# Cheng-Lin-Li/show-attend-and-tell

Hardware: AMD Instinct MI355X
Metric: training images/sec (higher is better)
Workload: dtype bf16; 1 GPU; model=vgg16_frozen+attention_lstm512, global_batch=32, seq_len=20, vocab=5000, parallelism=dp1

## Files before the change

### sat_amd/ops/csrc/bptt_fuse.hip

```cpp

#include "common.h"


__global__ void lstm_in_fuse_kernel(const bf16* __restrict__ pooled,
                                    const bf16* __restrict__ table,
                                    const int64_t* __restrict__ ids,
                                    const bf16* __restrict__ sth,
                                    const int64_t* __restrict__ seed_p,
                                    bf16* __restrict__ xh,
                                    int B, int D, int E, int H,
                                    float p, int salt) {
    const uint32_t seed = (uint32_t)(*seed_p);
    const int I = D + E;
    const int W = I + H;
    int64_t idx = (int64_t)blockIdx.x * blockDim.x + threadIdx.x;
    if (idx >= (int64_t)B * W) return;
    int b = idx / W, j = idx % W;
    if (j < D && pooled == nullptr) return;
    float val;
    if (j < I) {
        val = (j < D) ? bf2f(pooled[(int64_t)b * D + j])
                      : bf2f(table[ids[b] * E + (j - D)]);
        val *= drop_scale(seed, salt, (uint32_t)(b * I + j), p);
    } else {
        val = bf2f(sth[(int64_t)b * H + (j - I)]);
    }
    xh[idx] = f2bf(val);
}

void lstm_in_fuse(at::Tensor pooled, at::Tensor table, at::Tensor ids,
                  at::Tensor sth, at::Tensor seed, double p, int64_t salt,
                  at::Tensor xh) {
    int B = pooled.size(0), D = pooled.size(1), E = table.size(1),
        H = sth.size(1);
    int64_t n = (int64_t)B * (D + E + H);
    hipStream_t s = at::cuda::getCurrentCUDAStream();
    hipLaunchKernelGGL(lstm_in_fuse_kernel, dim3(cdiv(n, 256)), dim3(256),
                       0, s,
                       (const bf16*)pooled.data_ptr(),
                       (const bf16*)table.data_ptr(),
                       (const int64_t*)ids.data_ptr(),
                       (const bf16*)sth.data_ptr(),
                       (const int64_t*)seed.data_ptr(),
                       (bf16*)xh.data_ptr(), B, D, E, H,
                       (float)p, (int)salt);
    HIP_OK(hipGetLastError());
}

void lstm_in_tail(at::Tensor table, at::Tensor ids, at::Tensor sth,
                  at::Tensor seed, double p, int64_t salt, at::Tensor xh,
                  int64_t D) {
    int B = sth.size(0), E = table.size(1), H = sth.size(1);
    TORCH_CHECK(xh.is_contiguous() && xh.numel() == (int64_t)B * (D + E + H)
                && ids.numel() == B);
    int64_t n = (int64_t)B * (D + E + H);
    hipStream_t s = at::cuda::getCurrentCUDAStream();
    hipLaunchKernelGGL(lstm_in_fuse_kernel, dim3(cdiv(n, 256)), dim3(256),
                       0, s, (const bf16*)nullptr,
                       (const bf16*)table.data_ptr(),
                       (const int64_t*)ids.data_ptr(),
                       (const bf16*)sth.data_ptr(),
                       (const int64_t*)seed.data_ptr(),
                       (bf16*)xh.data_ptr(), B, (int)D, E, H,
                       (float)p, (int)salt);
    HIP_OK(hipGetLastError());
}


__global__ void expand_fuse_kernel(const bf16* __restrict__ h_raw,
                                   const bf16* __restrict__ pooled,
                                   const bf16* __restrict__ table,
                                   const int64_t* __restrict__ ids,
                                   const int64_t* __restrict__ seed_p,
                                   bf16* __restrict__ out_t,
                                   bf16* __restrict__ sth_t,
                                   bf16* __restrict__ expdrop,
                                   bf16* __restrict__ od_next,
                                   int B, int H, int D, int E,
                                   float p_lstm, float p_fc, int s) {
    const uint32_t seed = (uint32_t)(*seed_p);
    const int W = H + D + E;
    int64_t idx = (int64_t)blockIdx.x * blockDim.x + threadIdx.x;
    if (idx >= (int64_t)B * W) return;
    int b = idx / W, j = idx % W;
    float val;
    if (j < H) {
        float h = bf2f(h_raw[(int64_t)b * H + j]);
        uint32_t hidx = (uint32_t)(b * H + j);
        float ot = h * drop_scale(seed, s + 4, hidx, p_lstm);
        out_t[(int64_t)b * H + j] = f2bf(ot);
        sth_t[(int64_t)b * H + j] =
            f2bf(h * drop_scale(seed, s + 5, hidx, p_lstm));
        if (od_next != nullptr)
            od_next[(int64_t)b * H + j] =
                f2bf(ot * drop_scale(seed, s + 16 + 1, hidx, p_fc));
        val = ot;
    } else if (j < H + D) {
        val = bf2f(pooled[(int64_t)b * D + (j - H)]);
    } else {
        val = bf2f(table[ids[b] * E + (j - H - D)]);
    }
    expdrop[idx] = f2bf(val * drop_scale(seed, s + 6,
                                         (uint32_t)(b * W + j), p_fc));
}

std::vector<at::Tensor> expand_fuse(at::Tensor h_raw, at::Tensor pooled,
                                    at::Tensor table, at::Tensor ids,
                                    at::Tensor seed,
                                    at::Tensor expdrop, at::Tensor od_next,
                                    double p_lstm, double p_fc,
                                    int64_t s) {
    int B = h_raw.size(0), H = h_raw.size(1), D = pooled.size(1),
        E = table.size(1);
    auto out_t = at::empty_like(h_raw);
    auto sth_t = at::empty_like(h_raw);
    bf16* od_ptr = nullptr;
    if (od_next.defined() && od_next.numel() > 0)
        od_ptr = (bf16*)od_next.data_ptr();
    int64_t n = (int64_t)B * (H + D + E);
    hipStream_t st = at::cuda::getCurrentCUDAStream();
    hipLaunchKernelGGL(expand_fuse_kernel, dim3(cdiv(n, 256)), dim3(256),
                       0, st,
                       (const bf16*)h_raw.data_ptr(),
                       (const bf16*)pooled.data_ptr(),
                       (const bf16*)table.data_ptr(),
                       (const int64_t*)ids.data_ptr(),
                       (const int64_t*)seed.data_ptr(),
                       (bf16*)out_t.data_ptr(), (bf16*)sth_t.data_ptr(),
                       (bf16*)expdrop.data_ptr(), od_ptr,
                       B, H, D, E, (float)p_lstm, (float)p_fc, (int)s);
    HIP_OK(hipGetLastError());
    return {out_t, sth_t};
}


__global__ void dexp_fuse_kernel(const bf16* __restrict__ dexpd,
                                 const bf16* __restrict__ d_out_carry,
                                 const bf16* __restrict__ d_sth_carry,
                                 const int64_t* __restrict__ seed_p,
                                 bf16* __restrict__ dh_raw,
                                 bf16* __restrict__ dpool_dec,
                                 bf16* __restrict__ demb_dec,
                                 int B, int H, int D, int E,
                                 float p_fc, float p_lstm, int s) {
    const uint32_t seed = (uint32_t)(*seed_p);
    const int W = H + D + E;
    int64_t idx = (int64_t)blockIdx.x * blockDim.x + threadIdx.x;
    if (idx >= (int64_t)B * W) return;
    int b = idx / W, j = idx % W;
    float dexp = bf2f(dexpd[idx])
        * drop_scale(seed, s + 6, (uint32_t)(b * W + j), p_fc);
    if (j < H) {
        uint32_t hidx = (uint32_t)(b * H + j);
        float dout = dexp + bf2f(d_out_carry[(int64_t)b * H + j]);
        float dh = dout * drop_scale(seed, s + 4, hidx, p_lstm)
            + bf2f(d_sth_carry[(int64_t)b * H + j])
            * drop_scale(seed, s + 5, hidx, p_lstm);
        dh_raw[(int64_t)b * H + j] = f2bf(dh);
    } else if (j < H + D) {
        dpool_dec[(int64_t)b * D + (j - H)] = f2bf(dexp);
    } else {
        demb_dec[(int64_t)b * E + (j - H - D)] = f2bf(dexp);
    }
}

std::vector<at::Tensor> dexp_fuse(at::Tensor dexpd, at::Tensor d_out_carry,
                                  at::Tensor d_sth_carry, at::Tensor seed,
                                  double p_fc, double p_lstm, int64_t s,
                                  int64_t D, int64_t E) {
    int B = d_out_carry.size(0), H = d_out_carry.size(1);
    auto dh_raw = at::empty_like(d_out_carry);
    auto dpool = at::empty({B, D}, d_out_carry.options());
    auto demb = at::empty({B, E}, d_out_carry.options());
    int64_t n = (int64_t)B * (H + D + E);
    hipStream_t st = at::cuda::getCurrentCUDAStream();
    hipLaunchKernelGGL(dexp_fuse_kernel, dim3(cdiv(n, 256)), dim3(256),
                       0, st,
                       (const bf16*)dexpd.data_ptr(),
                       (const bf16*)d_out_carry.data_ptr(),
                       (const bf16*)d_sth_carry.data_ptr(),
                       (const int64_t*)seed.data_ptr(),
                       (bf16*)dh_raw.data_ptr(), (bf16*)dpool.data_ptr(),
                       (bf16*)demb.data_ptr(), B, H, (int)D, (int)E,
                       (float)p_fc, (float)p_lstm, (int)s);
    HIP_OK(hipGetLastError());
    return {dh_raw, dpool, demb};
}


__global__ void dx_fuse_kernel(const bf16* __restrict__ dxh,
                               const bf16* __restrict__ dpool_dec,
                               const bf16* __restrict__ demb_dec,
                               const int64_t* __restrict__ seed_p,
                               bf16* __restrict__ dpooled,
                               bf16* __restrict__ demb_out,
                               bf16* __restrict__ dsth,
                               int B, int D, int E, int H,
                               float p, int salt) {
    const uint32_t seed = (uint32_t)(*seed_p);
    const int I = D + E;
    const int W = I + H;
    int64_t idx = (int64_t)blockIdx.x * blockDim.x + threadIdx.x;
    if (idx >= (int64_t)B * W) return;
    int b = idx / W, j = idx % W;
    float g = bf2f(dxh[idx]);
    if (j < I) {
        g *= drop_scale(seed, salt, (uint32_t)(b * I + j), p);
        if (j < D)
            dpooled[(int64_t)b * D + j] =
                f2bf(g + bf2f(dpool_dec[(int64_t)b * D + j]));
        else
            demb_out[(int64_t)b * E + (j - D)] =
                f2bf(g + bf2f(demb_dec[(int64_t)b * E + (j - D)]));
    } else {
        dsth[(int64_t)b * H + (j - I)] = f2bf(g);
    }
}

std::vector<at::Tensor> dx_fuse(at::Tensor dxh, at::Tensor dpool_dec,
                                at::Tensor demb_dec, at::Tensor seed,
                                at::Tensor demb_out, double p,
                                int64_t salt, int64_t H) {
    int B = dpool_dec.size(0), D = dpool_dec.size(1), E = demb_dec.size(1);
    auto dpooled = at::empty_like(dpool_dec);
    auto dsth = at::empty({B, H}, dpool_dec.options());
    int64_t n = (int64_t)B * (D + E + H);
    hipStream_t st = at::cuda::getCurrentCUDAStream();
    hipLaunchKernelGGL(dx_fuse_kernel, dim3(cdiv(n, 256)), dim3(256),
                       0, st,
                       (const bf16*)dxh.data_ptr(),
                       (const bf16*)dpool_dec.data_ptr(),
                       (const bf16*)demb_dec.data_ptr(),
                       (const int64_t*)seed.data_ptr(),
                       (bf16*)dpooled.data_ptr(),
                       (bf16*)demb_out.data_ptr(),
                       (bf16*)dsth.data_ptr(),
                       B, D, E, (int)H, (float)p, (int)salt);
    HIP_OK(hipGetLastError());
    return {dpooled, dsth};
}


__global__ void hash_dropout_out_kernel(const bf16* __restrict__ x,
                                        const int64_t* __restrict__ seed_p,
                                        bf16* __restrict__ y,
                                        int64_t n, float p, int salt) {
    const uint32_t seed = (uint32_t)(*seed_p);
    int64_t idx = (int64_t)blockIdx.x * blockDim.x + threadIdx.x;
    if (idx >= n) return;
    y[idx] = f2bf(bf2f(x[idx])
                  * drop_scale(seed, salt, (uint32_t)idx, p));
}

void hash_dropout_out(at::Tensor x, at::Tensor seed, double p,
                      int64_t salt, at::Tensor out) {
    int64_t n = x.numel();
    hipStream_t s = at::cuda::getCurrentCUDAStream();
    hipLaunchKernelGGL(hash_dropout_out_kernel, dim3(cdiv(n, 256)),
                       dim3(256), 0, s,
                       (const bf16*)x.data_ptr(),
                       (const int64_t*)seed.data_ptr(),
                       (bf16*)out.data_ptr(), n, (float)p, (int)salt);
    HIP_OK(hipGetLastError());
}


__global__ void hash_dropout_steps_kernel(const bf16* __restrict__ x,
                                          const int64_t* __restrict__ seed_p,
                                          bf16* __restrict__ y,
                                          int64_t n, int T, float p,
                                          int salt_base, int salt_stride) {
    const uint32_t seed = (uint32_t)(*seed_p);
    int64_t i8 = ((int64_t)blockIdx.x * blockDim.x + threadIdx.x) * 8;
    int64_t total = n * T;
    int64_t stride = (int64_t)gridDim.x * blockDim.x * 8;
    for (; i8 < total; i8 += stride) {
        int t = (int)(i8 / n);
        int64_t j = i8 % n;
        int salt = salt_base + t * salt_stride;
        bf16x8 v = *(const bf16x8*)(x + j);
        bf16x8 o;
#pragma unroll
        for (int e = 0; e < 8; ++e)
            o[e] = f2bf(bf2f(v[e]) * drop_scale(seed, salt,
                                                (uint32_t)(j + e), p));
        *(bf16x8*)(y + i8) = o;
    }
}

at::Tensor hash_dropout_steps(at::Tensor x, at::Tensor seed, double p,
                              int64_t salt_base, int64_t salt_stride,
                              int64_t T) {
    int64_t n = x.numel();
    TORCH_CHECK(n % 8 == 0, "hash_dropout_steps needs numel % 8 == 0");
    auto y = at::empty({T, x.size(0), x.size(1)}, x.options());
    hipStream_t s = at::cuda::getCurrentCUDAStream();
    int blocks = (int)std::min<int64_t>(cdiv(n * T, 256 * 8), 16384);
    hipLaunchKernelGGL(hash_dropout_steps_kernel, dim3(blocks), dim3(256),
                       0, s,
                       (const bf16*)x.data_ptr(),
                       (const int64_t*)seed.data_ptr(),
                       (bf16*)y.data_ptr(), n, (int)T, (float)p,
                       (int)salt_base, (int)salt_stride);
    HIP_OK(hipGetLastError());
    return y;
}

__global__ void act_bwd_out_kernel(const bf16* __restrict__ dy,
                                   const bf16* __restrict__ y,
                                   bf16* __restrict__ dpre,
                                   int64_t n, int act) {
    int64_t idx = (int64_t)blockIdx.x * blockDim.x + threadIdx.x;
    if (idx >= n) return;
    float g = bf2f(dy[idx]);
    float yv = bf2f(y[idx]);
    if (act == 1) g *= (1.f - yv * yv);
    else if (act == 2) g *= (yv > 0.f ? 1.f : 0.f);
    dpre[idx] = f2bf(g);
}

void act_bwd_out(at::Tensor dy, at::Tensor y, int64_t act, at::Tensor out) {
    int64_t n = dy.numel();
    hipStream_t s = at::cuda::getCurrentCUDAStream();
    hipLaunchKernelGGL(act_bwd_out_kernel, dim3(cdiv(n, 256)), dim3(256),
                       0, s,
                       (const bf16*)dy.data_ptr(), (const bf16*)y.data_ptr(),
                       (bf16*)out.data_ptr(), n, (int)act);
    HIP_OK(hipGetLastError());
}

__global__ void act_bwd_f32_out_kernel(const float* __restrict__ dy,
                                       const bf16* __restrict__ y,
                                       bf16* __restrict__ dpre,
                                       int64_t n, int act) {
    int64_t idx = (int64_t)blockIdx.x * blockDim.x + threadIdx.x;
    if (idx >= n) return;
    float g = dy[idx];
    float yv = bf2f(y[idx]);
    if (act == 1) g *= (1.f - yv * yv);
    else if (act == 2) g *= (yv > 0.f ? 1.f : 0.f);
    dpre[idx] = f2bf(g);
}

void act_bwd_f32_out(at::Tensor dy, at::Tensor y, int64_t act,
                     at::Tensor out) {
    int64_t n = dy.numel();
    hipStream_t s = at::cuda::getCurrentCUDAStream();
    hipLaunchKernelGGL(act_bwd_f32_out_kernel, dim3(cdiv(n, 256)),
                       dim3(256), 0, s,
                       (const float*)dy.data_ptr(),
                       (const bf16*)y.data_ptr(),
                       (bf16*)out.data_ptr(), n, (int)act);
    HIP_OK(hipGetLastError());
}


__global__ void hash_dropout_slabs_kernel(const bf16* __restrict__ x,
                                          const int64_t* __restrict__ seed_p,
                                          bf16* __restrict__ y,
                                          int64_t slab_elems, int T,
                                          float p, int salt_base,
                                          int salt_stride) {
    const uint32_t seed = (uint32_t)(*seed_p);
    int64_t i8 = ((int64_t)blockIdx.x * blockDim.x + threadIdx.x) * 8;
    int64_t total = slab_elems * T;
    if (i8 >= total) return;
    int t = (int)(i8 / slab_elems);
    int64_t j = i8 % slab_elems;
    int salt = salt_base + t * salt_stride;
    bf16x8 v = *(const bf16x8*)(x + i8);
    bf16x8 o;
#pragma unroll
    for (int e = 0; e < 8; ++e)
        o[e] = f2bf(bf2f(v[e])
                    * drop_scale(seed, salt, (uint32_t)(j + e), p));
    *(bf16x8*)(y + i8) = o;
}

at::Tensor hash_dropout_slabs(at::Tensor x, at::Tensor seed, double p,
                              int64_t salt_base, int64_t salt_stride,
                              int64_t T) {
    if (p <= 0.0) return x;
    int64_t n = x.numel();
    int64_t slab = n / T;
    TORCH_CHECK(slab % 8 == 0 && n % T == 0);
    auto y = at::empty_like(x);
    hipStream_t s = at::cuda::getCurrentCUDAStream();
    hipLaunchKernelGGL(hash_dropout_slabs_kernel,
                       dim3(cdiv(n / 8, 256)), dim3(256), 0, s,
                       (const bf16*)x.data_ptr(),
                       (const int64_t*)seed.data_ptr(),
                       (bf16*)y.data_ptr(), slab, (int)T, (float)p,
                       (int)salt_base, (int)salt_stride);
    HIP_OK(hipGetLastError());
    return y;
}


__global__ void dexp_lstm_bwd_kernel(const bf16* __restrict__ dexpd,
                                     const bf16* __restrict__ d_out_carry,
                                     const bf16* __restrict__ d_sth_carry,
                                     const int64_t* __restrict__ seed_p,
                                     const bf16* __restrict__ gates,
                                     const bf16* __restrict__ c,
                                     const bf16* __restrict__ dc,
                                     bf16* __restrict__ dgates,
                                     bf16* __restrict__ dc_prev,
                                     bf16* __restrict__ dpool_dec,
                                     bf16* __restrict__ demb_dec,
                                     int B, int H, int D, int E,
                                     float p_fc, float p_lstm, int s,
                                     float fb,
                                     const float* __restrict__ carry_slabs,
                                     int carry_splitk, int carry_salt) {
    const uint32_t seed = (uint32_t)(*seed_p);
    const int W = H + D + E;
    int64_t idx = (int64_t)blockIdx.x * blockDim.x + threadIdx.x;
    if (idx >= (int64_t)B * W) return;
    int b = idx / W, j = idx % W;
    float dexp = bf2f(dexpd[idx])
        * drop_scale(seed, s + 6, (uint32_t)(b * W + j), p_fc);
    if (j < H) {
        uint32_t hidx = (uint32_t)(b * H + j);
        float doc;
        if (carry_slabs != nullptr) {
            float v = sum_slabs(carry_slabs, (int64_t)B * H,
                                (int64_t)b * H + j, carry_splitk);
            v *= drop_scale(seed, carry_salt, hidx, p_fc);
            doc = bf2f(f2bf(v));
        } else {
            doc = bf2f(d_out_carry[(int64_t)b * H + j]);
        }
        float dout = dexp + doc;
        float dhv = dout * drop_scale(seed, s + 4, hidx, p_lstm)
            + bf2f(d_sth_carry[(int64_t)b * H + j])
            * drop_scale(seed, s + 5, hidx, p_lstm);
        const bf16* gp = gates + (int64_t)b * 4 * H + j;
        float g[4], dg[4], dcp;
#pragma unroll
        for (int q = 0; q < 4; ++q) g[q] = bf2f(gp[q * H]);
        float dcv = (dc != nullptr) ? bf2f(dc[(int64_t)b * H + j]) : 0.f;
        lstm_cell_bwd(g, bf2f(c[(int64_t)b * H + j]), dhv, dcv, fb, dg,
                      dcp);
        bf16* dgp = dgates + (int64_t)b * 4 * H + j;
#pragma unroll
        for (int q = 0; q < 4; ++q) dgp[q * H] = f2bf(dg[q]);
        dc_prev[(int64_t)b * H + j] = f2bf(dcp);
    } else if (j < H + D) {
        dpool_dec[(int64_t)b * D + (j - H)] = f2bf(dexp);
    } else {
        demb_dec[(int64_t)b * E + (j - H - D)] = f2bf(dexp);
    }
}

static std::vector<at::Tensor> dexp_lstm_bwd_impl(
        at::Tensor dexpd, const bf16* carry_ptr, const float* slab_ptr,
        int carry_splitk, int64_t carry_salt, at::Tensor d_sth_carry,
        at::Tensor seed, at::Tensor gates, at::Tensor c_prev,
        at::Tensor dc, at::Tensor dgates_out, double p_fc, double p_lstm,
        int64_t s, int64_t D, int64_t E, double fb) {
    CHECK_GPU(dexpd); CHECK_BF16(dexpd);
    int B = d_sth_carry.size(0), H = d_sth_carry.size(1);
    TORCH_CHECK(dexpd.numel() == (int64_t)B * (H + D + E));
    TORCH_CHECK(dgates_out.numel() == (int64_t)B * 4 * H);
    auto dc_prev = at::empty({B, H}, dexpd.options());
    auto dpool_dec = at::empty({B, D}, dexpd.options());
    auto demb_dec = at::empty({B, E}, dexpd.options());
    const bf16* dc_ptr = nullptr;
    if (dc.defined() && dc.numel() > 0)
        dc_ptr = (const bf16*)dc.data_ptr();
    int64_t n = (int64_t)B * (H + D + E);
    hipStream_t st = at::cuda::getCurrentCUDAStream();
    hipLaunchKernelGGL(dexp_lstm_bwd_kernel, dim3(cdiv(n, 256)),
                       dim3(256), 0, st,
                       (const bf16*)dexpd.data_ptr(), carry_ptr,
                       (const bf16*)d_sth_carry.data_ptr(),
                       (const int64_t*)seed.data_ptr(),
                       (const bf16*)gates.data_ptr(),
                       (const bf16*)c_prev.data_ptr(), dc_ptr,
                       (bf16*)dgates_out.data_ptr(),
                       (bf16*)dc_prev.data_ptr(),
                       (bf16*)dpool_dec.data_ptr(),
                       (bf16*)demb_dec.data_ptr(),
                       B, H, (int)D, (int)E,
                       (float)p_fc, (float)p_lstm, (int)s, (float)fb,
                       slab_ptr, carry_splitk, (int)carry_salt);
    HIP_OK(hipGetLastError());
    return {dc_prev, dpool_dec, demb_dec};
}

std::vector<at::Tensor> dexp_lstm_bwd(at::Tensor dexpd,
                                      at::Tensor d_out_carry,
                                      at::Tensor d_sth_carry,
                                      at::Tensor seed, at::Tensor gates,
                                      at::Tensor c_prev, at::Tensor dc,
                                      at::Tensor dgates_out,
                                      double p_fc, double p_lstm,
                                      int64_t s, int64_t D, int64_t E,
                                      double fb) {
    TORCH_CHECK(d_out_carry.numel() == d_sth_carry.numel());
    return dexp_lstm_bwd_impl(dexpd, (const bf16*)d_out_carry.data_ptr(),
                              nullptr, 0, 0, d_sth_carry, seed, gates,
                              c_prev, dc, dgates_out, p_fc, p_lstm, s, D,
                              E, fb);
}

std::vector<at::Tensor> dexp_lstm_bwd_slabs(at::Tensor dexpd,
                                            at::Tensor carry_slabs,
                                            int64_t carry_salt,
                                            at::Tensor d_sth_carry,
                                            at::Tensor seed,
                                            at::Tensor gates,
                                            at::Tensor c_prev,
                                            at::Tensor dc,
                                            at::Tensor dgates_out,
                                            double p_fc, double p_lstm,
                                            int64_t s, int64_t D,
                                            int64_t E, double fb) {
    CHECK_GPU(carry_slabs); CHECK_CONTIG(carry_slabs);
    CHECK_F32(carry_slabs);
    TORCH_CHECK(carry_slabs.dim() == 3
                && carry_slabs.size(1) == d_sth_carry.size(0)
                && carry_slabs.size(2) == d_sth_carry.size(1),
                "carry slabs must be [splitk, B, H]");
    return dexp_lstm_bwd_impl(dexpd, nullptr,
                              (const float*)carry_slabs.data_ptr(),
                              (int)carry_slabs.size(0), carry_salt,
                              d_sth_carry, seed, gates, c_prev, dc,
                              dgates_out, p_fc, p_lstm, s, D, E, fb);
}
```

### sat_amd/ops/csrc/common.h

```cpp
#pragma once

#include <hip/hip_runtime.h>
#include <hip/hip_bf16.h>
#include <torch/extension.h>
#include <ATen/cuda/CUDAContext.h>

#define CHECK_GPU(x) TORCH_CHECK((x).is_cuda(), #x " must be on GPU")
#define CHECK_CONTIG(x) TORCH_CHECK((x).is_contiguous(), #x " must be contiguous")
#define CHECK_BF16(x) TORCH_CHECK((x).scalar_type() == at::kBFloat16, #x " must be bf16")
#define CHECK_F32(x) TORCH_CHECK((x).scalar_type() == at::kFloat, #x " must be fp32")

#define HIP_OK(expr) do { hipError_t _e = (expr); \
    TORCH_CHECK(_e == hipSuccess, "HIP error: ", hipGetErrorString(_e)); } while (0)

using bf16 = __bf16;
typedef __attribute__((ext_vector_type(8))) __bf16 bf16x8;
typedef __attribute__((ext_vector_type(4))) float floatx4;

static inline int cdiv(int64_t a, int64_t b) { return (int)((a + b - 1) / b); }

__device__ __forceinline__ float bf2f(bf16 v) { return (float)v; }
__device__ __forceinline__ bf16 f2bf(float v) { return (bf16)v; }

__device__ __forceinline__ float wave_sum(float v) {
    for (int off = 32; off > 0; off >>= 1)
        v += __shfl_down(v, off, 64);
    return v;
}

__device__ __forceinline__ float wave_max(float v) {
    for (int off = 32; off > 0; off >>= 1)
        v = fmaxf(v, __shfl_down(v, off, 64));
    return v;
}

__device__ __forceinline__ float sigmoidf(float x) {
    return 1.0f / (1.0f + __expf(-x));
}

__device__ __forceinline__ uint32_t mix3(uint32_t a, uint32_t b, uint32_t c) {
    uint32_t h = a * 0x9E3779B1u ^ b * 0x85EBCA77u ^ c * 0xC2B2AE3Du;
    h ^= h >> 16; h *= 0x7FEB352Du;
    h ^= h >> 15; h *= 0x846CA68Bu;
    h ^= h >> 16;
    return h;
}

__device__ __forceinline__ float drop_scale(uint32_t seed, int salt,
                                            uint32_t idx, float p) {
    if (p <= 0.f) return 1.f;
    uint32_t h = mix3(seed, (uint32_t)salt, idx);
    float u = (h >> 8) * (1.0f / 16777216.0f);
    return u >= p ? 1.0f / (1.0f - p) : 0.0f;
}

__device__ __forceinline__ void drop_scale8(uint32_t seed, int salt,
                                            uint32_t idx8, float p,
                                            float* sc) {
    if (p <= 0.f) {
#pragma unroll
        for (int e = 0; e < 8; ++e) sc[e] = 1.f;
        return;
    }
    uint32_t pq = (uint32_t)(p * 256.0f);
    float inv = 1.0f / (1.0f - p);
    uint32_t h1 = mix3(seed, (uint32_t)salt, idx8);
    uint32_t h2 = mix3(h1, (uint32_t)salt ^ 0xA5A5A5A5u, idx8);
#pragma unroll
    for (int e = 0; e < 4; ++e) {
        sc[e] = ((h1 >> (e * 8)) & 0xFFu) >= pq ? inv : 0.f;
        sc[4 + e] = ((h2 >> (e * 8)) & 0xFFu) >= pq ? inv : 0.f;
    }
}

struct LstmAct { float gi, gj, gf, go, cn; };

__device__ __forceinline__ LstmAct lstm_act(const float g[4], float cp,
                                            float fb) {
#pragma clang fp contract(off)
    LstmAct a;
    a.gi = sigmoidf(g[0]);
    a.gj = tanhf(g[1]);
    a.gf = sigmoidf(g[2] + fb);
    a.go = sigmoidf(g[3]);
    a.cn = fmaf(a.gi, a.gj, cp * a.gf);
    return a;
}

__device__ __forceinline__ void lstm_cell_fwd(const float g[4], float cp,
                                              float fb, float& cn,
                                              float& h) {
    LstmAct a = lstm_act(g, cp, fb);
    cn = a.cn;
    h = tanhf(a.cn) * a.go;
}

__device__ __forceinline__ void lstm_cell_bwd(const float g[4], float cp,
                                              float dhv, float dcv,
                                              float fb, float dg[4],
                                              float& dcp) {
#pragma clang fp contract(off)
    LstmAct a = lstm_act(g, cp, fb);
    float tc = tanhf(a.cn);
    float dct = fmaf(dhv * a.go, 1.f - tc * tc, dcv);
    dg[0] = dct * a.gj * a.gi * (1.f - a.gi);
    dg[1] = dct * a.gi * fmaf(-a.gj, a.gj, 1.f);
    dg[2] = dct * cp * a.gf * (1.f - a.gf);
    dg[3] = dhv * tc * a.go * (1.f - a.go);
    dcp = dct * a.gf;
}


struct PadPix { int pix, y, x; };

__device__ __forceinline__ PadPix pad_pix(int m, int H, int W) {
    int b = m / (H * W);
    int yx = m - b * (H * W);
    PadPix p;
    p.y = yx / W;
    p.x = yx - p.y * W;
    p.pix = (b * (H + 2) + p.y + 1) * (W + 2) + p.x + 1;
    return p;
}

__device__ __forceinline__ void pad_pix_next(PadPix& p, int H, int W) {
    const bool wx = (p.x + 1 == W);
    const bool wy = wx && (p.y + 1 == H);
    p.pix += 1 + (wx ? 2 : 0) + (wy ? 2 * (W + 2) : 0);
    p.y = wy ? 0 : (wx ? p.y + 1 : p.y);
    p.x = wx ? 0 : p.x + 1;
}

template <typename T>
__device__ __forceinline__ void pad_border_zero(bf16* p, int y, int x,
                                                int H, int W, int C) {
    const bool l = (x == 0), r = (x == W - 1);
    if (!(l || r || y == 0 || y == H - 1)) return;
    const int64_t rs = (int64_t)(W + 2) * C;
    const T z = {};
    if (l) *(T*)(p - C) = z;
    if (r) *(T*)(p + C) = z;
    if (y == 0) {
        *(T*)(p - rs) = z;
        if (l) *(T*)(p - rs - C) = z;
        if (r) *(T*)(p - rs + C) = z;
    }
    if (y == H - 1) {
        *(T*)(p + rs) = z;
        if (l) *(T*)(p + rs - C) = z;
        if (r) *(T*)(p + rs + C) = z;
    }
}

__device__ __forceinline__ void pad_border_run(bf16* out, int row0, int M,
                                               int H, int W, int C,
                                               const int (&cols)[4]) {
    if (row0 >= M) return;
    PadPix p = pad_pix(row0, H, W);
#pragma unroll 1
    for (int r = 0; r < 4 && row0 + r < M; ++r) {
        if (r) pad_pix_next(p, H, W);
        if (p.x == 0 || p.x == W - 1 || p.y == 0 || p.y == H - 1) {
            bf16* q = out + (int64_t)p.pix * C;
#pragma unroll 1
            for (int j = 0; j < 4; ++j)
                if (cols[j] < C)
                    pad_border_zero<bf16>(q + cols[j], p.y, p.x, H, W, C);
        }
    }
}

static inline at::Tensor nhwc_out(const at::Tensor& like, int64_t B,
                                  int64_t C, int64_t H, int64_t W,
                                  bool emit_pad,
                                  const c10::optional<at::Tensor>& out) {
    const int64_t Ho = emit_pad ? H + 2 : H, Wo = emit_pad ? W + 2 : W;
    TORCH_CHECK(B * Ho * Wo < (1LL << 31), "output has >= 2^31 pixels");
    if (out.has_value() && out->defined()) {
        CHECK_GPU(*out); CHECK_BF16(*out);
        TORCH_CHECK(out->dim() == 4 && out->size(0) == B
                    && out->size(1) == C && out->size(2) == Ho
                    && out->size(3) == Wo,
                    "out: expected [", B, ",", C, ",", Ho, ",", Wo, "]");
        TORCH_CHECK(out->is_contiguous(at::MemoryFormat::ChannelsLast),
                    "out must be channels_last");
        TORCH_CHECK(out->device() == like.device(),
                    "out must be on the input's device");
        return *out;
    }
    return at::empty({B, C, Ho, Wo},
                     like.options()
                         .memory_format(at::MemoryFormat::ChannelsLast));
}

__device__ __forceinline__ float sum_slabs(const float* __restrict__ Yf,
                                           int64_t n, int64_t off,
                                           int splitk) {
    float v = 0.f;
    for (int k = 0; k < splitk; ++k) v += Yf[k * n + off];
    return v;
}
```

### sat_amd/ops/csrc/gemm.hip

```cpp

#include "common.h"

at::Tensor dense_8p_fwd(at::Tensor x, at::Tensor w, at::Tensor bias,
                        int64_t act);
at::Tensor hash_dropout(at::Tensor x, at::Tensor seed, double p,
                        int64_t salt);

#define BK 64
#define LDS_STRIDE (BK + 8)

#define ACT_NONE 0
#define ACT_TANH 1
#define ACT_RELU 2

__device__ __forceinline__ float apply_act(float v, int act) {
    if (act == ACT_TANH) return tanhf(v);
    if (act == ACT_RELU) return fmaxf(v, 0.f);
    return v;
}


template <int WR, int WC, int FM, int FN>
__global__ __launch_bounds__(256)
void tiled_gemm_kernel(const bf16* __restrict__ A,
                       const bf16* __restrict__ W,
                       const bf16* __restrict__ bias,
                       bf16* __restrict__ Y,
                       int M, int N, int K, int act,
                       float* __restrict__ Yf, int kchunk) {
    constexpr int BM = WR * FM * 16;
    constexpr int BN = WC * FN * 16;
    __shared__ bf16 As[BM * LDS_STRIDE];
    __shared__ bf16 Bs[BN * LDS_STRIDE];

    const int tid = threadIdx.x;
    const int lane = tid & 63;
    const int wave = tid >> 6;
    const int wr = wave / WC;
    const int wc = wave % WC;

    const int bm = blockIdx.y * BM;
    const int bn = blockIdx.x * BN;

    floatx4 acc[FM][FN];
#pragma unroll
    for (int i = 0; i < FM; ++i)
#pragma unroll
        for (int j = 0; j < FN; ++j)
            acc[i][j] = floatx4{0.f, 0.f, 0.f, 0.f};

    const int lrow = lane & 15;
    const int kgrp = lane >> 4;

    constexpr int A_CHUNKS = BM * BK / 8 / 256;
    constexpr int B_CHUNKS = BN * BK / 8 / 256;

    int kbeg = 0, kend = K;
    if (Yf != nullptr) {
        kbeg = blockIdx.z * kchunk;
        kend = min(K, kbeg + kchunk);
    }
    for (int k0 = kbeg; k0 < kend; k0 += BK) {
#pragma unroll
        for (int i = 0; i < A_CHUNKS; ++i) {
            int q = tid + 256 * i;
            int row = q >> 3;
            int c8 = (q & 7) * 8;
            int gk = k0 + c8;
            bf16x8 v = {};
            int ga = bm + row;
            if (ga < M && gk + 8 <= K) {
                v = *(const bf16x8*)(A + (int64_t)ga * K + gk);
            } else if (ga < M) {
                for (int e = 0; e < 8; ++e)
                    if (gk + e < K) v[e] = A[(int64_t)ga * K + gk + e];
            }
            *(bf16x8*)(As + row * LDS_STRIDE + c8) = v;
        }
#pragma unroll
        for (int i = 0; i < B_CHUNKS; ++i) {
            int q = tid + 256 * i;
            int row = q >> 3;
            int c8 = (q & 7) * 8;
            int gk = k0 + c8;
            bf16x8 v = {};
            int gb = bn + row;
            if (gb < N && gk + 8 <= K) {
                v = *(const bf16x8*)(W + (int64_t)gb * K + gk);
            } else if (gb < N) {
                for (int e = 0; e < 8; ++e)
                    if (gk + e < K) v[e] = W[(int64_t)gb * K + gk + e];
            }
            *(bf16x8*)(Bs + row * LDS_STRIDE + c8) = v;
        }
        __syncthreads();

#pragma unroll
        for (int kk = 0; kk < BK / 32; ++kk) {
            bf16x8 a_frag[FM], b_frag[FN];
            const int kof = kk * 32 + kgrp * 8;
#pragma unroll
            for (int mi = 0; mi < FM; ++mi)
                a_frag[mi] = *(const bf16x8*)(
                    As + (wr * FM * 16 + mi * 16 + lrow) * LDS_STRIDE + kof);
#pragma unroll
            for (int ni = 0; ni < FN; ++ni)
                b_frag[ni] = *(const bf16x8*)(
                    Bs + (wc * FN * 16 + ni * 16 + lrow) * LDS_STRIDE + kof);
#pragma unroll
            for (int mi = 0; mi < FM; ++mi)
#pragma unroll
                for (int ni = 0; ni < FN; ++ni)
                    acc[mi][ni] = __builtin_amdgcn_mfma_f32_16x16x32_bf16(
                        a_frag[mi], b_frag[ni], acc[mi][ni], 0, 0, 0);
        }
        __syncthreads();
    }

    float* slab = (Yf != nullptr)
        ? Yf + (int64_t)blockIdx.z * M * N : nullptr;
#pragma unroll
    for (int ni = 0; ni < FN; ++ni) {
        int col = bn + wc * FN * 16 + ni * 16 + (lane & 15);
        float bv = (bias != nullptr && col < N) ? bf2f(bias[col]) : 0.f;
#pragma unroll
        for (int mi = 0; mi < FM; ++mi) {
#pragma unroll
            for (int r = 0; r < 4; ++r) {
                int row = bm + wr * FM * 16 + mi * 16 + (lane >> 4) * 4 + r;
                if (row < M && col < N) {
                    if (slab != nullptr)
                        slab[(int64_t)row * N + col] = acc[mi][ni][r];
                    else
                        Y[(int64_t)row * N + col] =
                            f2bf(apply_act(acc[mi][ni][r] + bv, act));
                }
            }
        }
    }
}


template <int RF, bool TANHA>
__global__ __launch_bounds__(256)
void skinny_gemm_kernel(const bf16* __restrict__ A,
                        const bf16* __restrict__ W,
                        const bf16* __restrict__ bias,
                        bf16* __restrict__ Y,
                        float* __restrict__ Yf,
                        int M, int N, int K, int act, int splitk,
                        const float* __restrict__ Af,
                        const bf16* __restrict__ Ay,
                        bf16* __restrict__ Apre) {
    const int lane = threadIdx.x & 63;
    const int wave = threadIdx.x >> 6;
    const int n0 = blockIdx.x * 64 + wave * 16;
    const bool active = (n0 < N);

    const int kq = blockIdx.y;
    const int kchunk = ((K / 32 + splitk - 1) / splitk) * 32;
    const int kbeg = kq * kchunk;
    const int kend = min(K, kbeg + kchunk);

    const int lrow = lane & 15;
    const int kgrp = lane >> 4;

    floatx4 acc[RF];
#pragma unroll
    for (int i = 0; i < RF; ++i)
        acc[i] = floatx4{0.f, 0.f, 0.f, 0.f};

    const bool wfull = (n0 + 16 <= N);
    if (active) {
        for (int k = kbeg; k < kend; k += 32) {
            const int kof = k + kgrp * 8;
            bf16x8 b_frag = {};
            if (kof + 8 <= K) {
                int gb = n0 + lrow;
                if (wfull || gb < N)
                    b_frag = *(const bf16x8*)(W + (int64_t)gb * K + kof);
            } else if (kof < K) {
                int gb = n0 + lrow;
                if (wfull || gb < N)
                    for (int e = 0; e < 8 && kof + e < K; ++e)
                        b_frag[e] = W[(int64_t)gb * K + kof + e];
            }
#pragma unroll
            for (int mi = 0; mi < RF; ++mi) {
                bf16x8 a0 = {};
                int ar = mi * 16 + lrow;
                if constexpr (TANHA) {
                    if (ar < M) {
                        const int64_t ao = (int64_t)ar * K + kof;
                        floatx4 g0 = *(const floatx4*)(Af + ao);
                        floatx4 g1 = *(const floatx4*)(Af + ao + 4);
                        bf16x8 yv = *(const bf16x8*)(Ay + ao);
#pragma unroll
                        for (int e = 0; e < 8; ++e) {
                            float y = bf2f(yv[e]);
                            float g = e < 4 ? g0[e] : g1[e - 4];
                            a0[e] = f2bf(g * (1.f - y * y));
                        }
                        if (blockIdx.x == 0 && wave == 0)
                            *(bf16x8*)(Apre + ao) = a0;
                    }
                } else
                if (kof + 8 <= K) {
                    if (ar < M)
                        a0 = *(const bf16x8*)(A + (int64_t)ar * K + kof);
                } else if (kof < K) {
                    if (ar < M)
                        for (int e = 0; e < 8 && kof + e < K; ++e)
                            a0[e] = A[(int64_t)ar * K + kof + e];
                }
                acc[mi] = __builtin_amdgcn_mfma_f32_16x16x32_bf16(
                    a0, b_frag, acc[mi], 0, 0, 0);
            }
        }
    }

    const int col = n0 + (lane & 15);
    if (!active || col >= N) return;
    if (Yf == nullptr) {
        float bv = (bias != nullptr) ? bf2f(bias[col]) : 0.f;
#pragma unroll
        for (int mi = 0; mi < RF; ++mi)
#pragma unroll
            for (int r = 0; r < 4; ++r) {
                int row = mi * 16 + (lane >> 4) * 4 + r;
                if (row < M)
                    Y[(int64_t)row * N + col] =
                        f2bf(apply_act(acc[mi][r] + bv, act));
            }
        return;
    }

    float* slab = Yf + (int64_t)kq * M * N;
#pragma unroll
    for (int mi = 0; mi < RF; ++mi)
#pragma unroll
        for (int r = 0; r < 4; ++r) {
            int row = mi * 16 + (lane >> 4) * 4 + r;
            if (row < M)
                slab[(int64_t)row * N + col] = acc[mi][r];
        }
}

__global__ void skinny_epilogue_kernel(const float* __restrict__ Yf,
                                       const bf16* __restrict__ bias,
                                       bf16* __restrict__ Y,
                                       int64_t n, int N, int act,
                                       int splitk) {
    int64_t idx = (int64_t)blockIdx.x * blockDim.x + threadIdx.x;
    if (idx >= n) return;
    float v = sum_slabs(Yf, n, idx, splitk);
    if (bias != nullptr) v += bf2f(bias[idx % N]);
    Y[idx] = f2bf(apply_act(v, act));
}

__global__ void dense_glds_kernel(const bf16* __restrict__ A,
                                  const bf16* __restrict__ W,
                                  const bf16* __restrict__ bias,
                                  bf16* __restrict__ Y,
                                  int M, int N, int K, int act);


static bool is_skinny(int64_t M, int64_t K) {
    return M <= 128 && K % 32 == 0;
}

struct SkinnyPlan { int nblocks, splitk; };

static SkinnyPlan skinny_plan(int64_t N, int64_t K) {
    int nblocks = cdiv(N, 64);
    int splitk = 1;
    while (nblocks * splitk < 192 && splitk < 8 &&
           (int)(K / 32) >= 2 * splitk)
        splitk *= 2;
    return {nblocks, splitk};
}

static void launch_skinny(hipStream_t stream, const at::Tensor& x,
                          const at::Tensor& w, const bf16* bias, bf16* y,
                          float* yf, int act, SkinnyPlan plan) {
    const int M = x.size(0), K = x.size(1), N = w.size(0);
    TORCH_CHECK(is_skinny(M, K),
                "skinny GEMM: M <= 128 and K % 32 == 0 only");
    auto kernel = M <= 32 ? skinny_gemm_kernel<2, false>
                : M <= 64 ? skinny_gemm_kernel<4, false>
                          : skinny_gemm_kernel<8, false>;
    hipLaunchKernelGGL(kernel, dim3(plan.nblocks, plan.splitk), dim3(256),
                       0, stream, (const bf16*)x.data_ptr(),
                       (const bf16*)w.data_ptr(), bias, y, yf, M, N, K,
                       act, plan.splitk, (const float*)nullptr,
                       (const bf16*)nullptr, (bf16*)nullptr);
}

at::Tensor dense_tanhbwd_slabs(at::Tensor dy, at::Tensor y, at::Tensor w,
                               at::Tensor dpre_out) {
    CHECK_GPU(dy); CHECK_CONTIG(dy); CHECK_F32(dy);
    CHECK_GPU(y); CHECK_CONTIG(y); CHECK_BF16(y);
    CHECK_GPU(w); CHECK_CONTIG(w); CHECK_BF16(w);
    CHECK_GPU(dpre_out); CHECK_CONTIG(dpre_out); CHECK_BF16(dpre_out);
    TORCH_CHECK(dy.dim() == 2 && w.dim() == 2);
    const int M = dy.size(0), K = dy.size(1), N = w.size(0);
    TORCH_CHECK(w.size(1) == K && y.numel() == dy.numel()
                && dpre_out.numel() == dy.numel(), "shape mismatch");
    TORCH_CHECK(is_skinny(M, K),
                "skinny GEMM: M <= 128 and K % 32 == 0 only");
    SkinnyPlan plan = skinny_plan(N, K);
    auto yf = at::empty({plan.splitk, M, N}, dy.options());
    auto kernel = M <= 32 ? skinny_gemm_kernel<2, true>
                : M <= 64 ? skinny_gemm_kernel<4, true>
                          : skinny_gemm_kernel<8, true>;
    hipStream_t stream = at::cuda::getCurrentCUDAStream();
    hipLaunchKernelGGL(kernel, dim3(plan.nblocks, plan.splitk), dim3(256),
                       0, stream, (const bf16*)nullptr,
                       (const bf16*)w.data_ptr(), (const bf16*)nullptr,
                       (bf16*)nullptr, (float*)yf.data_ptr(), M, N, K,
                       ACT_NONE, plan.splitk,
                       (const float*)dy.data_ptr(),
                       (const bf16*)y.data_ptr(),
                       (bf16*)dpre_out.data_ptr());
    HIP_OK(hipGetLastError());
    return yf;
}

static at::Tensor skinny_slabs(hipStream_t stream, const at::Tensor& x,
                               const at::Tensor& w) {
    SkinnyPlan plan = skinny_plan(w.size(0), x.size(1));
    auto yf = at::empty({plan.splitk, x.size(0), w.size(0)},
                        x.options().dtype(at::kFloat));
    launch_skinny(stream, x, w, nullptr, nullptr, (float*)yf.data_ptr(),
                  ACT_NONE, plan);
    return yf;
}

static void launch_tiled(hipStream_t stream, const at::Tensor& x,
                         const at::Tensor& w, const bf16* bias, bf16* y,
                         float* yf, int act, int splitk, int kchunk) {
    const int M = x.size(0), K = x.size(1), N = w.size(0);
    const bool narrow = N <= 512;
    auto kernel = narrow ? tiled_gemm_kernel<4, 1, 2, 4>
                         : tiled_gemm_kernel<2, 2, 4, 4>;
    dim3 grid(cdiv(N, narrow ? 64 : 128), cdiv(M, 128), splitk);
    hipLaunchKernelGGL(kernel, grid, dim3(256), 0, stream,
                       (const bf16*)x.data_ptr(),
                       (const bf16*)w.data_ptr(), bias, y, M, N, K, act,
                       yf, kchunk);
}

static void launch_epilogue(hipStream_t stream, const at::Tensor& yf,
                            const bf16* bias, at::Tensor& y, int act) {
    int64_t n = y.numel();
    hipLaunchKernelGGL(skinny_epilogue_kernel, dim3(cdiv(n, 256)),
                       dim3(256), 0, stream, (const float*)yf.data_ptr(),
                       bias, (bf16*)y.data_ptr(), n, (int)y.size(1), act,
                       (int)yf.size(0));
}

at::Tensor dense_fwd(at::Tensor x, at::Tensor w, at::Tensor bias,
                     int64_t act) {
    CHECK_GPU(x); CHECK_CONTIG(x); CHECK_BF16(x);
    CHECK_GPU(w); CHECK_CONTIG(w); CHECK_BF16(w);
    TORCH_CHECK(x.dim() == 2 && w.dim() == 2, "dense_fwd expects 2-D inputs");
    const int64_t M = x.size(0), K = x.size(1), N = w.size(0);
    TORCH_CHECK(w.size(1) == K, "weight inner dim mismatch");
    TORCH_CHECK(K % 8 == 0, "K must be a multiple of 8 (bf16x8 loads)");
    const bf16* bias_ptr = nullptr;
    if (bias.defined() && bias.numel() > 0) {
        CHECK_GPU(bias); CHECK_CONTIG(bias); CHECK_BF16(bias);
        TORCH_CHECK(bias.numel() == N, "bias size mismatch");
        bias_ptr = (const bf16*)bias.data_ptr();
    }
    const bool skinny = is_skinny(M, K);
    if (!skinny && M >= 16384 && N >= 256 && N % 8 == 0 && K % 64 == 0
        && K >= 128) {
        return dense_8p_fwd(x, w, bias_ptr != nullptr ? bias : at::Tensor(),
                            act);
    }
    auto y = at::empty({M, N}, x.options());
    hipStream_t stream = at::cuda::getCurrentCUDAStream();

    if (skinny) {
        SkinnyPlan plan = skinny_plan(N, K);
        if (plan.splitk == 1) {
            launch_skinny(stream, x, w, bias_ptr, (bf16*)y.data_ptr(),
                          nullptr, (int)act, plan);
        } else {
            auto yf = skinny_slabs(stream, x, w);
            launch_epilogue(stream, yf, bias_ptr, y, (int)act);
        }
    } else if (M >= 16384 && N % 128 == 0 && K % 64 == 0) {
        dim3 grid(cdiv(N, 128), cdiv(M, 128));
        hipLaunchKernelGGL(dense_glds_kernel, grid, dim3(256), 0,
                           stream,
                           (const bf16*)x.data_ptr(),
                           (const bf16*)w.data_ptr(), bias_ptr,
                           (bf16*)y.data_ptr(), (int)M, (int)N, (int)K,
                           (int)act);
    } else {
        int tiles = cdiv(N, N <= 512 ? 64 : 128) * cdiv(M, 128);
        int splitk = 1;
        while (tiles * splitk < 160 && splitk < 8
               && K >= 128 * 2 * splitk)
            splitk *= 2;
        int kchunk = cdiv(cdiv(K, splitk), 64) * 64;
        splitk = cdiv(K, kchunk);
        if (splitk == 1) {
            launch_tiled(stream, x, w, bias_ptr, (bf16*)y.data_ptr(),
                         nullptr, (int)act, 1, kchunk);
        } else {
            auto yf = at::empty({splitk, M, N},
                                x.options().dtype(at::kFloat));
            launch_tiled(stream, x, w, bias_ptr, (bf16*)y.data_ptr(),
                         (float*)yf.data_ptr(), (int)act, splitk, kchunk);
            launch_epilogue(stream, yf, bias_ptr, y, (int)act);
        }
    }
    HIP_OK(hipGetLastError());
    return y;
}


__global__ void skinny_epilogue_drop_kernel(
        const float* __restrict__ Yf, bf16* __restrict__ Y,
        const int64_t* __restrict__ seed_p, int64_t n, int splitk,
        float p, int salt) {
    int64_t idx = (int64_t)blockIdx.x * blockDim.x + threadIdx.x;
    if (idx >= n) return;
    float v = sum_slabs(Yf, n, idx, splitk);
    v *= drop_scale((uint32_t)(*seed_p), salt, (uint32_t)idx, p);
    Y[idx] = f2bf(v);
}

at::Tensor dense_fwd_drop(at::Tensor x, at::Tensor w, at::Tensor seed,
                          double p, int64_t salt) {
    CHECK_GPU(x); CHECK_CONTIG(x); CHECK_BF16(x);
    CHECK_GPU(w); CHECK_CONTIG(w); CHECK_BF16(w);
    int64_t M = x.size(0), K = x.size(1), N = w.size(0);
    if (p <= 0.0 || !is_skinny(M, K)) {
        auto y = dense_fwd(x, w, at::Tensor(), ACT_NONE);
        return p > 0.0 ? hash_dropout(y, seed, p, salt) : y;
    }
    auto y = at::empty({M, N}, x.options());
    hipStream_t stream = at::cuda::getCurrentCUDAStream();
    auto yf = skinny_slabs(stream, x, w);
    int64_t n = M * N;
    hipLaunchKernelGGL(skinny_epilogue_drop_kernel,
                       dim3(cdiv(n, 256)), dim3(256), 0, stream,
                       (const float*)yf.data_ptr(), (bf16*)y.data_ptr(),
                       (const int64_t*)seed.data_ptr(), n,
                       (int)yf.size(0), (float)p, (int)salt);
    HIP_OK(hipGetLastError());
    return y;
}

at::Tensor slab_epilogue_drop(at::Tensor yf, at::Tensor seed, double p,
                              int64_t salt) {
    CHECK_GPU(yf); CHECK_CONTIG(yf); CHECK_F32(yf);
    TORCH_CHECK(yf.dim() == 3, "slabs must be [splitk, M, N]");
    auto y = at::empty({yf.size(1), yf.size(2)},
                       yf.options().dtype(at::kBFloat16));
    int64_t n = y.numel();
    hipStream_t stream = at::cuda::getCurrentCUDAStream();
    hipLaunchKernelGGL(skinny_epilogue_drop_kernel,
                       dim3(cdiv(n, 256)), dim3(256), 0, stream,
                       (const float*)yf.data_ptr(), (bf16*)y.data_ptr(),
                       (const int64_t*)seed.data_ptr(), n,
                       (int)yf.size(0), (float)p, (int)salt);
    HIP_OK(hipGetLastError());
    return y;
}


__device__ __forceinline__ void sum_gates(const float* __restrict__ Yf,
                                          const bf16* __restrict__ bias,
                                          bf16* __restrict__ gates,
                                          int B, int H, int b, int hh,
                                          int splitk, float g[4]) {
    int64_t n = (int64_t)B * 4 * H;
#pragma unroll
    for (int q = 0; q < 4; ++q) {
        int64_t off = (int64_t)b * 4 * H + q * H + hh;
        float acc = sum_slabs(Yf, n, off, splitk);
        if (bias != nullptr) acc += bf2f(bias[q * H + hh]);
        gates[off] = f2bf(acc);
        g[q] = acc;
    }
}

__global__ void skinny_epi_lstm_kernel(const float* __restrict__ Yf,
                                       const bf16* __restrict__ bias,
                                       const bf16* __restrict__ c_prev,
                                       bf16* __restrict__ gates,
                                       bf16* __restrict__ h_out,
                                       bf16* __restrict__ c_out,
                                       int B, int H, int splitk,
                                       float fb) {
    int idx = blockIdx.x * blockDim.x + threadIdx.x;
    if (idx >= B * H) return;
    float g[4], cn, h;
    sum_gates(Yf, bias, gates, B, H, idx / H, idx % H, splitk, g);
    lstm_cell_fwd(g, bf2f(c_prev[idx]), fb, cn, h);
    h_out[idx] = f2bf(h);
    c_out[idx] = f2bf(cn);
}

std::vector<at::Tensor> dense_lstm_fwd(at::Tensor xh, at::Tensor wl,
                                       at::Tensor bl, at::Tensor c_prev,
                                       double fb) {
    int64_t M = xh.size(0), N = wl.size(0);
    int B = c_prev.size(0), H = c_prev.size(1);
    TORCH_CHECK(M == B && N == 4 * H);
    auto gates = at::empty({M, N}, xh.options());
    auto h_out = at::empty_like(c_prev);
    auto c_out = at::empty_like(c_prev);
    hipStream_t s = at::cuda::getCurrentCUDAStream();
    auto yf = skinny_slabs(s, xh, wl);
    hipLaunchKernelGGL(skinny_epi_lstm_kernel,
                       dim3(cdiv(B * H, 256)), dim3(256), 0, s,
                       (const float*)yf.data_ptr(),
                       (const bf16*)bl.data_ptr(),
                       (const bf16*)c_prev.data_ptr(),
                       (bf16*)gates.data_ptr(), (bf16*)h_out.data_ptr(),
                       (bf16*)c_out.data_ptr(), B, H, (int)yf.size(0),
                       (float)fb);
    HIP_OK(hipGetLastError());
    return {gates, h_out, c_out};
}



__global__ __launch_bounds__(256)
void dense_glds_kernel(const bf16* __restrict__ A,
                       const bf16* __restrict__ W,
                       const bf16* __restrict__ bias,
                       bf16* __restrict__ Y,
                       int M, int N, int K, int act) {
    constexpr int BM = 128, BN = 128, BKc = 64;
    __shared__ bf16 lds[2 * BM * BKc];
    bf16* As = lds;
    bf16* Bs = lds + BM * BKc;

    const int tid = threadIdx.x;
    const int lane = tid & 63;
    const int wave = tid >> 6;
    const int wr = wave >> 1, wc = wave & 1;
    const int bm = blockIdx.y * BM;
    const int bn = blockIdx.x * BN;

    const bf16* aSrc[4];
    const bf16* wSrc[4];
    const int ci8 = (lane & 7) * 8;
#pragma unroll
    for (int i = 0; i < 4; ++i) {
        int r = wave * 32 + i * 8 + (lane >> 3);
        int swz = (r & 4) ? 16 : 0;
        int ga = bm + r;
        if (ga >= M) ga = M - 1;
        aSrc[i] = A + (int64_t)ga * K + (ci8 ^ swz);
        int gb = bn + r;
        if (gb >= N) gb = N - 1;
        wSrc[i] = W + (int64_t)gb * K + (ci8 ^ swz);
    }

    floatx4 acc[4][4];
#pragma unroll
    for (int i = 0; i < 4; ++i)
#pragma unroll
        for (int j = 0; j < 4; ++j)
            acc[i][j] = floatx4{0.f, 0.f, 0.f, 0.f};

    const int lrow = lane & 15;
    const int kgrp = lane >> 4;

    for (int k0 = 0; k0 < K; k0 += BKc) {
#pragma unroll
        for (int i = 0; i < 4; ++i) {
            __builtin_amdgcn_global_load_lds(
                (const __attribute__((address_space(1))) uint32_t*)
                    (aSrc[i] + k0),
                (__attribute__((address_space(3))) uint32_t*)
                    (As + (wave * 32 + i * 8) * BKc),
                16, 0, 0);
            __builtin_amdgcn_global_load_lds(
                (const __attribute__((address_space(1))) uint32_t*)
                    (wSrc[i] + k0),
                (__attribute__((address_space(3))) uint32_t*)
                    (Bs + (wave * 32 + i * 8) * BKc),
                16, 0, 0);
        }
        __syncthreads();

#pragma unroll
        for (int kk = 0; kk < 2; ++kk) {
            bf16x8 a_frag[4], b_frag[4];
            const int kof = kk * 32 + kgrp * 8;
#pragma unroll
            for (int mi = 0; mi < 4; ++mi) {
                int r = wr * 64 + mi * 16 + lrow;
                a_frag[mi] = *(const bf16x8*)(
                    As + r * BKc + (kof ^ ((r & 4) ? 16 : 0)));
            }
#pragma unroll
            for (int ni = 0; ni < 4; ++ni) {
                int r = wc * 64 + ni * 16 + lrow;
                b_frag[ni] = *(const bf16x8*)(
                    Bs + r * BKc + (kof ^ ((r & 4) ? 16 : 0)));
            }
#pragma unroll
            for (int mi = 0; mi < 4; ++mi)
#pragma unroll
                for (int ni = 0; ni < 4; ++ni)
                    acc[mi][ni] = __builtin_amdgcn_mfma_f32_16x16x32_bf16(
                        a_frag[mi], b_frag[ni], acc[mi][ni], 0, 0, 0);
        }
        __syncthreads();
    }

#pragma unroll
    for (int ni = 0; ni < 4; ++ni) {
        int col = bn + wc * 64 + ni * 16 + (lane & 15);
        float bv = (bias != nullptr && col < N) ? bf2f(bias[col]) : 0.f;
#pragma unroll
        for (int mi = 0; mi < 4; ++mi) {
#pragma unroll
            for (int r = 0; r < 4; ++r) {
                int row = bm + wr * 64 + mi * 16 + (lane >> 4) * 4 + r;
                if (row < M && col < N) {
                    float vv = acc[mi][ni][r] + bv;
                    Y[(int64_t)row * N + col] = f2bf(apply_act(vv, act));
                }
            }
        }
    }
}


__global__ void skinny_epi_dx_kernel(const float* __restrict__ Yf,
                                     const bf16* __restrict__ dpool_dec,
                                     const bf16* __restrict__ demb_dec,
                                     const int64_t* __restrict__ seed_p,
                                     bf16* __restrict__ dpooled,
                                     bf16* __restrict__ demb_out,
                                     bf16* __restrict__ dsth,
                                     int64_t n, int splitk,
                                     int B, int D, int E, int H,
                                     float p, int salt) {
    const uint32_t seed = (uint32_t)(*seed_p);
    const int I = D + E;
    const int W = I + H;
    int64_t idx = (int64_t)blockIdx.x * blockDim.x + threadIdx.x;
    if (idx >= n) return;
    float g = sum_slabs(Yf, n, idx, splitk);
    int b = (int)(idx / W), j = (int)(idx % W);
    if (j < I) {
        g *= drop_scale(seed, salt, (uint32_t)(b * I + j), p);
        if (j < D)
            dpooled[(int64_t)b * D + j] =
                f2bf(g + bf2f(dpool_dec[(int64_t)b * D + j]));
        else
            demb_out[(int64_t)b * E + (j - D)] =
                f2bf(g + bf2f(demb_dec[(int64_t)b * E + (j - D)]));
    } else {
        dsth[(int64_t)b * H + (j - I)] = f2bf(g);
    }
}

std::vector<at::Tensor> dense_dx_fuse(at::Tensor dgates, at::Tensor wl_t,
                                      at::Tensor dpool_dec,
                                      at::Tensor demb_dec,
                                      at::Tensor seed,
                                      at::Tensor demb_out,
                                      double p, int64_t salt,
                                      int64_t D, int64_t E, int64_t H) {
    CHECK_GPU(dgates); CHECK_CONTIG(dgates); CHECK_BF16(dgates);
    CHECK_GPU(wl_t); CHECK_CONTIG(wl_t); CHECK_BF16(wl_t);
    int64_t M = dgates.size(0), N = wl_t.size(0);
    TORCH_CHECK(N == D + E + H);
    auto dpooled = at::empty({M, D}, dgates.options());
    auto dsth = at::empty({M, H}, dgates.options());
    hipStream_t stream = at::cuda::getCurrentCUDAStream();
    auto yf = skinny_slabs(stream, dgates, wl_t);
    int64_t n = M * N;
    hipLaunchKernelGGL(skinny_epi_dx_kernel, dim3(cdiv(n, 256)),
                       dim3(256), 0, stream,
                       (const float*)yf.data_ptr(),
                       (const bf16*)dpool_dec.data_ptr(),
                       (const bf16*)demb_dec.data_ptr(),
                       (const int64_t*)seed.data_ptr(),
                       (bf16*)dpooled.data_ptr(),
                       (bf16*)demb_out.data_ptr(),
                       (bf16*)dsth.data_ptr(),
                       n, (int)yf.size(0), (int)M, (int)D, (int)E, (int)H,
                       (float)p, (int)salt);
    HIP_OK(hipGetLastError());
    return {dpooled, dsth};
}


__global__ void skinny_epi_lstm_expand_kernel(
        const float* __restrict__ Yf, const bf16* __restrict__ bias,
        const bf16* __restrict__ c_prev,
        const bf16* __restrict__ pooled,
        const bf16* __restrict__ table,
        const int64_t* __restrict__ ids,
        const int64_t* __restrict__ seed_p,
        bf16* __restrict__ gates, bf16* __restrict__ c_out,
        bf16* __restrict__ sth_t, bf16* __restrict__ expdrop,
        bf16* __restrict__ od_next,
        int B, int H, int D, int E, int splitk,
        float fb, float p_lstm, float p_fc, int s,
        const int64_t* __restrict__ next_ids,
        bf16* __restrict__ xh_next) {
    const uint32_t seed = (uint32_t)(*seed_p);
    const int W = H + D + E;
    const int I = D + E;
    int64_t idx = (int64_t)blockIdx.x * blockDim.x + threadIdx.x;
    if (idx >= (int64_t)B * W) return;
    int b = idx / W, j = idx % W;
    float val;
    if (j < H) {
        float g[4], cn, h;
        sum_gates(Yf, bias, gates, B, H, b, j, splitk, g);
        lstm_cell_fwd(g, bf2f(c_prev[(int64_t)b * H + j]), fb, cn, h);
        c_out[(int64_t)b * H + j] = f2bf(cn);
        uint32_t hidx = (uint32_t)(b * H + j);
        float ot = h * drop_scale(seed, s + 4, hidx, p_lstm);
        bf16 sth = f2bf(h * drop_scale(seed, s + 5, hidx, p_lstm));
        sth_t[(int64_t)b * H + j] = sth;
        if (xh_next != nullptr)
            xh_next[(int64_t)b * W + I + j] = sth;
        if (od_next != nullptr)
            od_next[(int64_t)b * H + j] =
                f2bf(ot * drop_scale(seed, s + 16 + 1, hidx, p_fc));
        val = ot;
    } else if (j < H + D) {
        val = bf2f(pooled[(int64_t)b * D + (j - H)]);
    } else {
        int e = j - H - D;
        val = bf2f(table[ids[b] * E + e]);
        if (xh_next != nullptr)
            xh_next[(int64_t)b * W + D + e] =
                f2bf(bf2f(table[next_ids[b] * E + e])
                     * drop_scale(seed, s + 16 + 3,
                                  (uint32_t)(b * I + D + e), p_lstm));
    }
    expdrop[idx] = f2bf(val * drop_scale(seed, s + 6,
                                         (uint32_t)(b * W + j), p_fc));
}

static std::vector<at::Tensor> dense_lstm_expand_impl(
        at::Tensor xh, at::Tensor wl, at::Tensor bl, at::Tensor c_prev,
        at::Tensor pooled, at::Tensor table, at::Tensor ids,
        at::Tensor seed, at::Tensor expdrop, at::Tensor od_next,
        double fb, double p_lstm, double p_fc, int64_t s,
        const int64_t* next_ids_ptr, bf16* xh_next_ptr) {
    int64_t M = xh.size(0), N = wl.size(0);
    int B = c_prev.size(0), H = c_prev.size(1);
    int D = pooled.size(1), E = table.size(1);
    TORCH_CHECK(M == B && N == 4 * H);
    auto gates = at::empty({M, N}, xh.options());
    auto c_out = at::empty({B, H}, xh.options());
    auto sth_t = at::empty({B, H}, xh.options());
    hipStream_t stream = at::cuda::getCurrentCUDAStream();
    auto yf = skinny_slabs(stream, xh, wl);
    const bf16* bias_ptr = nullptr;
    if (bl.defined() && bl.numel() > 0)
        bias_ptr = (const bf16*)bl.data_ptr();
    bf16* od_ptr = nullptr;
    if (od_next.defined() && od_next.numel() > 0)
        od_ptr = (bf16*)od_next.data_ptr();
    int64_t n = (int64_t)B * (H + D + E);
    hipLaunchKernelGGL(skinny_epi_lstm_expand_kernel,
                       dim3(cdiv(n, 256)), dim3(256), 0, stream,
                       (const float*)yf.data_ptr(), bias_ptr,
                       (const bf16*)c_prev.data_ptr(),
                       (const bf16*)pooled.data_ptr(),
                       (const bf16*)table.data_ptr(),
                       (const int64_t*)ids.data_ptr(),
                       (const int64_t*)seed.data_ptr(),
                       (bf16*)gates.data_ptr(),
                       (bf16*)c_out.data_ptr(),
                       (bf16*)sth_t.data_ptr(),
                       (bf16*)expdrop.data_ptr(), od_ptr,
                       B, H, D, E, (int)yf.size(0),
                       (float)fb, (float)p_lstm, (float)p_fc, (int)s,
                       next_ids_ptr, xh_next_ptr);
    HIP_OK(hipGetLastError());
    return {gates, c_out, sth_t};
}

std::vector<at::Tensor> dense_lstm_expand_fwd(
        at::Tensor xh, at::Tensor wl, at::Tensor bl, at::Tensor c_prev,
        at::Tensor pooled, at::Tensor table, at::Tensor ids,
        at::Tensor seed, at::Tensor expdrop, at::Tensor od_next,
        double fb, double p_lstm, double p_fc, int64_t s) {
    return dense_lstm_expand_impl(xh, wl, bl, c_prev, pooled, table, ids,
                                  seed, expdrop, od_next, fb, p_lstm, p_fc,
                                  s, nullptr, nullptr);
}

std::vector<at::Tensor> dense_lstm_expand_xh_fwd(
        at::Tensor xh, at::Tensor wl, at::Tensor bl, at::Tensor c_prev,
        at::Tensor pooled, at::Tensor table, at::Tensor ids,
        at::Tensor seed, at::Tensor expdrop, at::Tensor od_next,
        double fb, double p_lstm, double p_fc, int64_t s,
        at::Tensor next_ids, at::Tensor xh_next) {
    const int64_t* nid = nullptr;
    bf16* xn = nullptr;
    if (xh_next.defined() && xh_next.numel() > 0) {
        CHECK_GPU(xh_next); CHECK_CONTIG(xh_next); CHECK_BF16(xh_next);
        CHECK_GPU(next_ids); CHECK_CONTIG(next_ids);
        TORCH_CHECK(next_ids.scalar_type() == at::kLong
                    && next_ids.numel() == c_prev.size(0));
        TORCH_CHECK(xh_next.numel() == c_prev.size(0)
                    * (c_prev.size(1) + pooled.size(1) + table.size(1)));
        nid = (const int64_t*)next_ids.data_ptr();
        xn = (bf16*)xh_next.data_ptr();
    }
    return dense_lstm_expand_impl(xh, wl, bl, c_prev, pooled, table, ids,
                                  seed, expdrop, od_next, fb, p_lstm, p_fc,
                                  s, nid, xn);
}
```

### sat_amd/ops/csrc/kernels.hip

```cpp

#include "common.h"


__global__ void lstm_pw_fwd_kernel(const bf16* __restrict__ gates,
                                   const bf16* __restrict__ c,
                                   bf16* __restrict__ h_out,
                                   bf16* __restrict__ c_out,
                                   int B, int H, float fb) {
    int idx = blockIdx.x * blockDim.x + threadIdx.x;
    if (idx >= B * H) return;
    int b = idx / H, hh = idx % H;
    const bf16* gp = gates + (int64_t)b * 4 * H + hh;
    float g[4];
#pragma unroll
    for (int q = 0; q < 4; ++q) g[q] = bf2f(gp[q * H]);
    float cn, h;
    lstm_cell_fwd(g, bf2f(c[idx]), fb, cn, h);
    h_out[idx] = f2bf(h);
    c_out[idx] = f2bf(cn);
}

__global__ void lstm_pw_bwd_kernel(const bf16* __restrict__ gates,
                                   const bf16* __restrict__ c,
                                   const bf16* __restrict__ dh,
                                   const bf16* __restrict__ dc,
                                   bf16* __restrict__ dgates,
                                   bf16* __restrict__ dc_prev,
                                   int B, int H, float fb) {
    int idx = blockIdx.x * blockDim.x + threadIdx.x;
    if (idx >= B * H) return;
    int b = idx / H, hh = idx % H;
    const bf16* gp = gates + (int64_t)b * 4 * H + hh;
    float g[4], dg[4], dcp;
#pragma unroll
    for (int q = 0; q < 4; ++q) g[q] = bf2f(gp[q * H]);
    float dcv = (dc != nullptr) ? bf2f(dc[idx]) : 0.f;
    lstm_cell_bwd(g, bf2f(c[idx]), bf2f(dh[idx]), dcv, fb, dg, dcp);
    bf16* dgp = dgates + (int64_t)b * 4 * H + hh;
#pragma unroll
    for (int q = 0; q < 4; ++q) dgp[q * H] = f2bf(dg[q]);
    dc_prev[idx] = f2bf(dcp);
}

std::vector<at::Tensor> lstm_pointwise_fwd(at::Tensor gates, at::Tensor c,
                                           double fb) {
    CHECK_GPU(gates); CHECK_CONTIG(gates); CHECK_BF16(gates);
    CHECK_GPU(c); CHECK_CONTIG(c); CHECK_BF16(c);
    int B = c.size(0), H = c.size(1);
    TORCH_CHECK(gates.size(0) == B && gates.size(1) == 4 * H);
    auto h_out = at::empty_like(c);
    auto c_out = at::empty_like(c);
    int n = B * H;
    hipStream_t s = at::cuda::getCurrentCUDAStream();
    hipLaunchKernelGGL(lstm_pw_fwd_kernel, dim3(cdiv(n, 256)), dim3(256), 0, s,
                       (const bf16*)gates.data_ptr(), (const bf16*)c.data_ptr(),
                       (bf16*)h_out.data_ptr(), (bf16*)c_out.data_ptr(),
                       B, H, (float)fb);
    HIP_OK(hipGetLastError());
    return {h_out, c_out};
}

std::vector<at::Tensor> lstm_pointwise_bwd_out(at::Tensor gates,
                                               at::Tensor c, at::Tensor dh,
                                               at::Tensor dc, double fb,
                                               at::Tensor dgates_out) {
    CHECK_GPU(gates); CHECK_CONTIG(gates); CHECK_BF16(gates);
    int B = c.size(0), H = c.size(1);
    at::Tensor dgates;
    if (dgates_out.defined() && dgates_out.numel() > 0)
        dgates = dgates_out;
    else
        dgates = at::empty_like(gates);
    auto dc_prev = at::empty_like(c);
    const bf16* dc_ptr = nullptr;
    if (dc.defined() && dc.numel() > 0) dc_ptr = (const bf16*)dc.data_ptr();
    int n = B * H;
    hipStream_t s = at::cuda::getCurrentCUDAStream();
    hipLaunchKernelGGL(lstm_pw_bwd_kernel, dim3(cdiv(n, 256)), dim3(256), 0, s,
                       (const bf16*)gates.data_ptr(), (const bf16*)c.data_ptr(),
                       (const bf16*)dh.data_ptr(), dc_ptr,
                       (bf16*)dgates.data_ptr(), (bf16*)dc_prev.data_ptr(),
                       B, H, (float)fb);
    HIP_OK(hipGetLastError());
    return {dgates, dc_prev};
}

std::vector<at::Tensor> lstm_pointwise_bwd(at::Tensor gates, at::Tensor c,
                                           at::Tensor dh, at::Tensor dc,
                                           double fb) {
    return lstm_pointwise_bwd_out(gates, c, dh, dc, fb, at::Tensor());
}


__global__ void act_bwd_kernel(const bf16* __restrict__ dy,
                               const bf16* __restrict__ y,
                               bf16* __restrict__ dpre,
                               int64_t n, int act) {
    int64_t idx = (int64_t)blockIdx.x * blockDim.x + threadIdx.x;
    if (idx >= n) return;
    float g = bf2f(dy[idx]);
    float yv = bf2f(y[idx]);
    if (act == 1) g *= (1.f - yv * yv);
    else if (act == 2) g *= (yv > 0.f ? 1.f : 0.f);
    dpre[idx] = f2bf(g);
}

at::Tensor act_bwd(at::Tensor dy, at::Tensor y, int64_t act) {
    CHECK_GPU(dy); CHECK_CONTIG(dy); CHECK_BF16(dy);
    CHECK_GPU(y); CHECK_CONTIG(y); CHECK_BF16(y);
    auto dpre = at::empty_like(dy);
    int64_t n = dy.numel();
    hipStream_t s = at::cuda::getCurrentCUDAStream();
    hipLaunchKernelGGL(act_bwd_kernel, dim3(cdiv(n, 256)), dim3(256), 0, s,
                       (const bf16*)dy.data_ptr(), (const bf16*)y.data_ptr(),
                       (bf16*)dpre.data_ptr(), n, (int)act);
    HIP_OK(hipGetLastError());
    return dpre;
}


#define MAX_L 1024


__global__ void hash_dropout_kernel(const bf16* __restrict__ x,
                                    const int64_t* __restrict__ seed_p,
                                    bf16* __restrict__ y,
                                    int64_t n, float p, int salt) {
    const uint32_t seed = (uint32_t)(*seed_p);
    int64_t idx = (int64_t)blockIdx.x * blockDim.x + threadIdx.x;
    int64_t stride = (int64_t)gridDim.x * blockDim.x;
    for (int64_t i = idx * 8; i < n; i += stride * 8) {
        if (i + 8 <= n) {
            bf16x8 v = *(const bf16x8*)(x + i);
            bf16x8 o;
#pragma unroll
            for (int e = 0; e < 8; ++e)
                o[e] = f2bf(bf2f(v[e]) *
                            drop_scale(seed, salt, (uint32_t)(i + e), p));
            *(bf16x8*)(y + i) = o;
        } else {
            for (int64_t j = i; j < n; ++j)
                y[j] = f2bf(bf2f(x[j]) *
                            drop_scale(seed, salt, (uint32_t)j, p));
        }
    }
}

at::Tensor hash_dropout(at::Tensor x, at::Tensor seed, double p,
                        int64_t salt) {
    CHECK_GPU(x); CHECK_CONTIG(x); CHECK_BF16(x);
    if (p <= 0.0) return x;
    auto y = at::empty_like(x);
    int64_t n = x.numel();
    int blocks = (int)std::min<int64_t>(cdiv(n, 256 * 8), 4096);
    hipStream_t s = at::cuda::getCurrentCUDAStream();
    hipLaunchKernelGGL(hash_dropout_kernel, dim3(blocks), dim3(256), 0, s,
                       (const bf16*)x.data_ptr(),
                       (const int64_t*)seed.data_ptr(),
                       (bf16*)y.data_ptr(), n, (float)p, (int)salt);
    HIP_OK(hipGetLastError());
    return y;
}


__global__ void attn_scores_fused_kernel(
        const bf16* __restrict__ t1, const bf16* __restrict__ t2,
        const bf16* __restrict__ v, const int64_t* __restrict__ seed_p,
        bf16* __restrict__ tdrop, float* __restrict__ logits,
        int B, int L, int A, float p, int salt) {
    const uint32_t seed = (uint32_t)(*seed_p);
    int row = blockIdx.x * 4 + (threadIdx.x >> 6);
    if (row >= B * L) return;
    int lane = threadIdx.x & 63;
    int b = row / L;
    const bf16* t1r = t1 + (int64_t)row * A;
    const bf16* t2r = t2 + (int64_t)b * A;
    bf16* tdr = tdrop + (int64_t)row * A;
    float acc = 0.f;
    for (int a0 = lane * 8; a0 + 8 <= A; a0 += 64 * 8) {
        bf16x8 x1 = *(const bf16x8*)(t1r + a0);
        bf16x8 x2 = *(const bf16x8*)(t2r + a0);
        bf16x8 vv = *(const bf16x8*)(v + a0);
        bf16x8 out;
        float sc[8];
        drop_scale8(seed, salt, (uint32_t)((row * A + a0) >> 3), p, sc);
#pragma unroll
        for (int e = 0; e < 8; ++e) {
            float t = (bf2f(x1[e]) + bf2f(x2[e])) * sc[e];
            out[e] = f2bf(t);
            acc += t * bf2f(vv[e]);
        }
        *(bf16x8*)(tdr + a0) = out;
    }
    acc = wave_sum(acc);
    if (lane == 0) logits[row] = acc;
}

std::vector<at::Tensor> attn_scores_fused(at::Tensor t1, at::Tensor t2,
                                          at::Tensor v, at::Tensor seed,
                                          double p, int64_t salt,
                                          int64_t L) {
    CHECK_GPU(t1); CHECK_CONTIG(t1); CHECK_BF16(t1);
    CHECK_GPU(t2); CHECK_CONTIG(t2); CHECK_BF16(t2);
    CHECK_GPU(v); CHECK_CONTIG(v); CHECK_BF16(v);
    int A = t1.size(1);
    int rows = t1.size(0);
    int B = rows / (int)L;
    TORCH_CHECK(A % 8 == 0 && rows % L == 0);
    auto tdrop = at::empty_like(t1);
    auto logits = at::empty({B, (int)L},
                            t1.options().dtype(at::kFloat));
    hipStream_t s = at::cuda::getCurrentCUDAStream();
    hipLaunchKernelGGL(attn_scores_fused_kernel, dim3(cdiv(rows, 4)),
                       dim3(256), 0, s,
                       (const bf16*)t1.data_ptr(),
                       (const bf16*)t2.data_ptr(),
                       (const bf16*)v.data_ptr(),
                       (const int64_t*)seed.data_ptr(),
                       (bf16*)tdrop.data_ptr(), (float*)logits.data_ptr(),
                       B, (int)L, A, (float)p, (int)salt);
    HIP_OK(hipGetLastError());
    return {tdrop, logits};
}


__global__ void attn_pool_bwd_p1_kernel(
        const bf16* __restrict__ ctx, const float* __restrict__ alpha,
        const bf16* __restrict__ dpooled,
        float* __restrict__ sbuf, bf16* __restrict__ dctx,
        int L, int D) {
    int b = blockIdx.x;
    int nchunk = gridDim.y;
    int lchunk = (L + nchunk - 1) / nchunk;
    int l0 = blockIdx.y * lchunk;
    int l1 = min(L, l0 + lchunk);
    int wid = threadIdx.x >> 6, lane = threadIdx.x & 63;
    const bf16* cb = ctx + (int64_t)b * L * D;
    const bf16* dp = dpooled + (int64_t)b * D;

    for (int l = l0 + wid; l < l1; l += 4) {
        float acc = 0.f;
        float a = alpha[(int64_t)b * L + l];
        for (int d0 = lane * 8; d0 + 8 <= D; d0 += 64 * 8) {
            bf16x8 cv = *(const bf16x8*)(cb + (int64_t)l * D + d0);
            bf16x8 dv = *(const bf16x8*)(dp + d0);
            if (dctx != nullptr) {
                bf16x8 out;
#pragma unroll
                for (int e = 0; e < 8; ++e) {
                    float dpe = bf2f(dv[e]);
                    acc += bf2f(cv[e]) * dpe;
                    out[e] = f2bf(a * dpe);
                }
                *(bf16x8*)(dctx + (int64_t)b * L * D + (int64_t)l * D + d0)
                    = out;
            } else {
#pragma unroll
                for (int e = 0; e < 8; ++e)
                    acc += bf2f(cv[e]) * bf2f(dv[e]);
            }
        }
        acc = wave_sum(acc);
        if (lane == 0) sbuf[(int64_t)b * L + l] = acc;
    }
}

__global__ void attn_pool_bwd_p2_kernel(
        const float* __restrict__ alpha, const float* __restrict__ dalpha,
        const float* __restrict__ sbuf, float* __restrict__ dlogits,
        int L) {
    __shared__ float red[4];
    int b = blockIdx.x;
    int tid = threadIdx.x;
    float part = 0.f;
    for (int l = tid; l < L; l += blockDim.x) {
        float da = sbuf[(int64_t)b * L + l];
        if (dalpha != nullptr) da += dalpha[(int64_t)b * L + l];
        part += alpha[(int64_t)b * L + l] * da;
    }
    part = wave_sum(part);
    if ((tid & 63) == 0) red[tid >> 6] = part;
    __syncthreads();
    float dot = red[0] + red[1] + red[2] + red[3];
    for (int l = tid; l < L; l += blockDim.x) {
        float da = sbuf[(int64_t)b * L + l];
        if (dalpha != nullptr) da += dalpha[(int64_t)b * L + l];
        dlogits[(int64_t)b * L + l] =
            alpha[(int64_t)b * L + l] * (da - dot);
    }
}

std::vector<at::Tensor> attn_pool_bwd(at::Tensor ctx, at::Tensor alpha,
                                      at::Tensor dalpha, at::Tensor dpooled,
                                      bool need_dctx) {
    CHECK_GPU(ctx); CHECK_CONTIG(ctx); CHECK_BF16(ctx);
    CHECK_GPU(alpha); CHECK_CONTIG(alpha); CHECK_F32(alpha);
    int B = ctx.size(0), L = ctx.size(1), D = ctx.size(2);
    TORCH_CHECK(L <= MAX_L && D % 8 == 0);
    auto dlogits = at::empty({B, L}, alpha.options());
    auto sbuf = at::empty({B, L}, alpha.options());
    at::Tensor dctx;
    bf16* dctx_ptr = nullptr;
    if (need_dctx) {
        dctx = at::empty_like(ctx);
        dctx_ptr = (bf16*)dctx.data_ptr();
    } else {
        dctx = at::empty({0}, ctx.options());
    }
    const float* dalpha_ptr = nullptr;
    if (dalpha.defined() && dalpha.numel() > 0)
        dalpha_ptr = (const float*)dalpha.data_ptr();
    hipStream_t s = at::cuda::getCurrentCUDAStream();
    hipLaunchKernelGGL(attn_pool_bwd_p1_kernel, dim3(B, 8), dim3(256), 0, s,
                       (const bf16*)ctx.data_ptr(),
                       (const float*)alpha.data_ptr(),
                       (const bf16*)dpooled.data_ptr(),
                       (float*)sbuf.data_ptr(), dctx_ptr, L, D);
    hipLaunchKernelGGL(attn_pool_bwd_p2_kernel, dim3(B), dim3(256), 0, s,
                       (const float*)alpha.data_ptr(), dalpha_ptr,
                       (const float*)sbuf.data_ptr(),
                       (float*)dlogits.data_ptr(), L);
    HIP_OK(hipGetLastError());
    return {dlogits, dctx};
}


template <int NCH>
__global__ void attn_scores_bwd_kernel(
        const bf16* __restrict__ tdrop, const bf16* __restrict__ v,
        const float* __restrict__ dlogits,
        const int64_t* __restrict__ seed_p,
        bf16* __restrict__ dt1, float* __restrict__ dt2,
        float* __restrict__ dvf,
        const bf16* __restrict__ t1y,
        int B, int L, int A, int lchunk, float p, int salt) {
    __shared__ float sdv[4][NCH * 512];
    __shared__ float sd2[4][NCH * 512];
    const uint32_t seed = (uint32_t)(*seed_p);
    int nchunk = (L + lchunk - 1) / lchunk;
    int b = blockIdx.x / nchunk;
    int l0 = (blockIdx.x % nchunk) * lchunk;
    int l1 = min(L, l0 + lchunk);
    int wid = threadIdx.x >> 6, lane = threadIdx.x & 63;

    float dv_acc[NCH][8] = {};
    float dt2_acc[NCH][8] = {};

    for (int l = l0 + wid; l < l1; l += 4) {
        int64_t row = (int64_t)b * L + l;
        float dl = dlogits[row];
#pragma unroll
        for (int ch = 0; ch < NCH; ++ch) {
            int a0 = ch * 512 + lane * 8;
            bf16x8 td = *(const bf16x8*)(tdrop + row * A + a0);
            bf16x8 vv = *(const bf16x8*)(v + a0);
            bf16x8 o;
            float sc[8];
            drop_scale8(seed, salt, (uint32_t)((row * A + a0) >> 3), p, sc);
            bf16x8 yv = {};
            if (t1y != nullptr)
                yv = *(const bf16x8*)(t1y + row * A + a0);
#pragma unroll
            for (int e = 0; e < 8; ++e) {
                dv_acc[ch][e] += bf2f(td[e]) * dl;
                float dt = dl * bf2f(vv[e]) * sc[e];
                dt2_acc[ch][e] += dt;
                if (t1y != nullptr) {
                    float y = bf2f(yv[e]);
                    dt *= (1.f - y * y);
                }
                o[e] = f2bf(dt);
            }
            *(bf16x8*)(dt1 + row * A + a0) = o;
        }
    }
#pragma unroll
    for (int ch = 0; ch < NCH; ++ch) {
        int a0 = ch * 512 + lane * 8;
#pragma unroll
        for (int e = 0; e < 8; ++e) {
            sdv[wid][a0 + e] = dv_acc[ch][e];
            sd2[wid][a0 + e] = dt2_acc[ch][e];
        }
    }
    __syncthreads();
    for (int a = threadIdx.x; a < A; a += (int)blockDim.x) {
        float dv_s = sdv[0][a] + sdv[1][a] + sdv[2][a] + sdv[3][a];
        float d2_s = sd2[0][a] + sd2[1][a] + sd2[2][a] + sd2[3][a];
        atomicAdd(dvf + a, dv_s);
        atomicAdd(dt2 + (int64_t)b * A + a, d2_s);
    }
}

static std::vector<at::Tensor> attn_scores_bwd_impl(
        at::Tensor tdrop, at::Tensor v, at::Tensor dlogits,
        at::Tensor seed, double p, int64_t salt, int64_t L,
        at::Tensor dv_acc, at::Tensor t1y, at::Tensor dt1_out,
        at::Tensor dt2_out) {
    CHECK_GPU(tdrop); CHECK_CONTIG(tdrop); CHECK_BF16(tdrop);
    int rows = tdrop.size(0), A = tdrop.size(1);
    TORCH_CHECK(A % 512 == 0 && A <= 2048,
                "attn_scores_bwd requires A % 512 == 0, A <= 2048");
    int B = rows / (int)L;
    at::Tensor dt1;
    if (dt1_out.defined() && dt1_out.numel() > 0) {
        TORCH_CHECK(dt1_out.numel() == tdrop.numel());
        dt1 = dt1_out;
    } else {
        dt1 = at::empty_like(tdrop);
    }
    const bf16* t1y_ptr = nullptr;
    if (t1y.defined() && t1y.numel() > 0) {
        TORCH_CHECK(t1y.numel() == tdrop.numel());
        t1y_ptr = (const bf16*)t1y.data_ptr();
    }
    at::Tensor dt2;
    if (dt2_out.defined() && dt2_out.numel() > 0) {
        CHECK_GPU(dt2_out); CHECK_CONTIG(dt2_out); CHECK_F32(dt2_out);
        TORCH_CHECK(dt2_out.numel() == (int64_t)B * A);
        dt2 = dt2_out;
    } else {
        dt2 = at::zeros({B, A}, tdrop.options().dtype(at::kFloat));
    }
    at::Tensor dvf;
    if (dv_acc.defined() && dv_acc.numel() > 0)
        dvf = dv_acc;
    else
        dvf = at::zeros({A}, tdrop.options().dtype(at::kFloat));
    int lchunk = ((int)L + 7) / 8;
    int nchunk = ((int)L + lchunk - 1) / lchunk;
    hipStream_t s = at::cuda::getCurrentCUDAStream();
#define LAUNCH_SB(NCH) \
    hipLaunchKernelGGL((attn_scores_bwd_kernel<NCH>), dim3(B * nchunk), \
                       dim3(256), 0, s, \
                       (const bf16*)tdrop.data_ptr(), \
                       (const bf16*)v.data_ptr(), \
                       (const float*)dlogits.data_ptr(), \
                       (const int64_t*)seed.data_ptr(), \
                       (bf16*)dt1.data_ptr(), (float*)dt2.data_ptr(), \
                       (float*)dvf.data_ptr(), t1y_ptr, \
                       B, (int)L, A, lchunk, (float)p, (int)salt)
    switch (A / 512) {
        case 1: LAUNCH_SB(1); break;
        case 2: LAUNCH_SB(2); break;
        case 3: LAUNCH_SB(3); break;
        default: LAUNCH_SB(4); break;
    }
#undef LAUNCH_SB
    HIP_OK(hipGetLastError());
    return {dt1, dt2, dvf};
}

std::vector<at::Tensor> attn_scores_bwd_tanh(
        at::Tensor tdrop, at::Tensor v, at::Tensor dlogits,
        at::Tensor seed, double p, int64_t salt, int64_t L,
        at::Tensor dv_acc, at::Tensor t1y, at::Tensor dt1_out) {
    return attn_scores_bwd_impl(tdrop, v, dlogits, seed, p, salt, L,
                                dv_acc, t1y, dt1_out, at::Tensor());
}

std::vector<at::Tensor> attn_scores_bwd_acc(at::Tensor tdrop, at::Tensor v,
                                            at::Tensor dlogits,
                                            at::Tensor seed, double p,
                                            int64_t salt, int64_t L,
                                            at::Tensor dv_acc) {
    return attn_scores_bwd_tanh(tdrop, v, dlogits, seed, p, salt, L,
                                dv_acc, at::Tensor(), at::Tensor());
}

std::vector<at::Tensor> attn_scores_bwd_step(
        at::Tensor tdrop, at::Tensor v, at::Tensor dlogits,
        at::Tensor seed, double p, int64_t salt, int64_t L,
        at::Tensor dv_acc, at::Tensor t1y, at::Tensor dt1_out,
        at::Tensor dt2_out) {
    return attn_scores_bwd_impl(tdrop, v, dlogits, seed, p, salt, L,
                                dv_acc, t1y, dt1_out, dt2_out);
}

std::vector<at::Tensor> attn_scores_bwd(at::Tensor tdrop, at::Tensor v,
                                        at::Tensor dlogits, at::Tensor seed,
                                        double p, int64_t salt, int64_t L) {
    return attn_scores_bwd_acc(tdrop, v, dlogits, seed, p, salt, L,
                               at::Tensor());
}

__global__ void attn_softmax_kernel(const float* __restrict__ logits,
                                    float* __restrict__ alpha, int L) {
    __shared__ float sa[MAX_L];
    __shared__ float red[8];
    int b = blockIdx.x;
    int tid = threadIdx.x;
    float lmax = -1e30f;
    for (int l = tid; l < L; l += blockDim.x) {
        float x = logits[(int64_t)b * L + l];
        sa[l] = x;
        lmax = fmaxf(lmax, x);
    }
    lmax = wave_max(lmax);
    if ((tid & 63) == 0) red[tid >> 6] = lmax;
    __syncthreads();
    float m = -1e30f;
    for (int w = 0; w < (int)(blockDim.x >> 6); ++w) m = fmaxf(m, red[w]);
    __syncthreads();
    float lsum = 0.f;
    for (int l = tid; l < L; l += blockDim.x) {
        float e = __expf(sa[l] - m);
        sa[l] = e;
        lsum += e;
    }
    lsum = wave_sum(lsum);
    if ((tid & 63) == 0) red[tid >> 6] = lsum;
    __syncthreads();
    float z = 0.f;
    for (int w = 0; w < (int)(blockDim.x >> 6); ++w) z += red[w];
    float inv = 1.0f / z;
    for (int l = tid; l < L; l += blockDim.x)
        alpha[(int64_t)b * L + l] = sa[l] * inv;
}

__global__ void attn_pool_sum_kernel(const bf16* __restrict__ ctx,
                                     const float* __restrict__ alpha,
                                     bf16* __restrict__ pooled,
                                     int L, int D) {
    __shared__ float sa[MAX_L];
    __shared__ float part[16][128 + 4];
    int b = blockIdx.x;
    int d0 = blockIdx.y * 128;
    int tid = threadIdx.x;
    for (int l = tid; l < L; l += blockDim.x)
        sa[l] = alpha[(int64_t)b * L + l];
    __syncthreads();
    int dg = tid & 15;
    int lg = tid >> 4;
    int d = d0 + dg * 8;
    float acc[8] = {};
    if (d < D) {
        const bf16* cb = ctx + (int64_t)b * L * D;
        for (int l = lg; l < L; l += 16) {
            bf16x8 cv = *(const bf16x8*)(cb + (int64_t)l * D + d);
            float a = sa[l];
#pragma unroll
            for (int e = 0; e < 8; ++e) acc[e] += a * bf2f(cv[e]);
        }
    }
#pragma unroll
    for (int e = 0; e < 8; ++e) part[lg][dg * 8 + e] = acc[e];
    __syncthreads();
    if (tid < 128 && d0 + tid < D) {
        float s = 0.f;
#pragma unroll
        for (int g = 0; g < 16; ++g) s += part[g][tid];
        pooled[(int64_t)b * D + d0 + tid] = f2bf(s);
    }
}

__global__ void attn_pool_fused_kernel(const bf16* __restrict__ ctx,
                                       const float* __restrict__ logits,
                                       float* __restrict__ alpha,
                                       bf16* __restrict__ pooled,
                                       int L, int D,
                                       bf16* __restrict__ xh,
                                       const int64_t* __restrict__ seed_p,
                                       int xh_stride, int I, float p,
                                       int salt) {
    __shared__ float sa[MAX_L];
    __shared__ float red[8];
    __shared__ float part[16][128 + 4];
    int b = blockIdx.x;
    int d0 = blockIdx.y * 128;
    int tid = threadIdx.x;

    float lmax = -1e30f;
    for (int l = tid; l < L; l += blockDim.x) {
        float x = logits[(int64_t)b * L + l];
        sa[l] = x;
        lmax = fmaxf(lmax, x);
    }
    lmax = wave_max(lmax);
    if ((tid & 63) == 0) red[tid >> 6] = lmax;
    __syncthreads();
    float m = -1e30f;
    for (int w = 0; w < (int)(blockDim.x >> 6); ++w)
        m = fmaxf(m, red[w]);
    __syncthreads();
    float lsum = 0.f;
    for (int l = tid; l < L; l += blockDim.x) {
        float e = __expf(sa[l] - m);
        sa[l] = e;
        lsum += e;
    }
    lsum = wave_sum(lsum);
    if ((tid & 63) == 0) red[tid >> 6] = lsum;
    __syncthreads();
    float z = 0.f;
    for (int w = 0; w < (int)(blockDim.x >> 6); ++w) z += red[w];
    float inv = 1.0f / z;
    __syncthreads();
    for (int l = tid; l < L; l += blockDim.x) {
        sa[l] *= inv;
        if (blockIdx.y == 0)
            alpha[(int64_t)b * L + l] = sa[l];
    }
    __syncthreads();

    int dg = tid & 15;
    int lg = tid >> 4;
    int d = d0 + dg * 8;
    float acc[8] = {};
    if (d < D) {
        const bf16* cb = ctx + (int64_t)b * L * D;
        for (int l = lg; l < L; l += 16) {
            bf16x8 cv = *(const bf16x8*)(cb + (int64_t)l * D + d);
            float a = sa[l];
#pragma unroll
            for (int e = 0; e < 8; ++e) acc[e] += a * bf2f(cv[e]);
        }
    }
#pragma unroll
    for (int e = 0; e < 8; ++e) part[lg][dg * 8 + e] = acc[e];
    __syncthreads();
    if (tid < 128 && d0 + tid < D) {
        float ssum = 0.f;
#pragma unroll
        for (int g = 0; g < 16; ++g) ssum += part[g][tid];
        bf16 pv = f2bf(ssum);
        pooled[(int64_t)b * D + d0 + tid] = pv;
        if (xh != nullptr) {
            int d = d0 + tid;
            xh[(int64_t)b * xh_stride + d] =
                f2bf(bf2f(pv) * drop_scale((uint32_t)(*seed_p), salt,
                                           (uint32_t)(b * I + d), p));
        }
    }
}

static std::vector<at::Tensor> attn_pool_fwd_impl(
        at::Tensor ctx, at::Tensor logits, bf16* xh_ptr,
        const int64_t* seed_ptr, int xh_stride, int I, double p,
        int64_t salt) {
    CHECK_GPU(ctx); CHECK_CONTIG(ctx); CHECK_BF16(ctx);
    CHECK_GPU(logits); CHECK_CONTIG(logits); CHECK_F32(logits);
    int B = ctx.size(0), L = ctx.size(1), D = ctx.size(2);
    TORCH_CHECK(L <= MAX_L, "attention locations exceed LDS stage");
    TORCH_CHECK(logits.numel() == (int64_t)B * L);
    auto alpha = at::empty({B, L}, ctx.options().dtype(at::kFloat));
    auto pooled = at::empty({B, D}, ctx.options());
    hipStream_t s = at::cuda::getCurrentCUDAStream();
    hipLaunchKernelGGL(attn_pool_fused_kernel, dim3(B, cdiv(D, 128)),
                       dim3(256), 0, s,
                       (const bf16*)ctx.data_ptr(),
                       (const float*)logits.data_ptr(),
                       (float*)alpha.data_ptr(),
                       (bf16*)pooled.data_ptr(), L, D,
                       xh_ptr, seed_ptr, xh_stride, I, (float)p,
                       (int)salt);
    HIP_OK(hipGetLastError());
    return {alpha, pooled};
}

std::vector<at::Tensor> attn_pool_fwd(at::Tensor ctx, at::Tensor logits) {
    return attn_pool_fwd_impl(ctx, logits, nullptr, nullptr, 0, 0, 0.0, 0);
}

std::vector<at::Tensor> attn_pool_fwd_xh(at::Tensor ctx, at::Tensor logits,
                                         at::Tensor seed, double p,
                                         int64_t salt, at::Tensor xh,
                                         int64_t I) {
    CHECK_GPU(xh); CHECK_CONTIG(xh); CHECK_BF16(xh);
    CHECK_GPU(seed);
    TORCH_CHECK(xh.dim() == 2 && xh.size(0) == ctx.size(0)
                && I >= ctx.size(2) && xh.size(1) >= I,
                "xh must be [B, I + H] with I >= D");
    return attn_pool_fwd_impl(ctx, logits, (bf16*)xh.data_ptr(),
                              (const int64_t*)seed.data_ptr(),
                              (int)xh.size(1), (int)I, p, salt);
}


__global__ void embedding_fwd_kernel(const int64_t* __restrict__ ids,
                                     const bf16* __restrict__ table,
                                     bf16* __restrict__ out,
                                     int B, int E) {
    int idx = blockIdx.x * blockDim.x + threadIdx.x;
    if (idx >= B * E) return;
    int b = idx / E, e = idx % E;
    out[idx] = table[ids[b] * E + e];
}

__global__ void embedding_bwd_kernel(const int64_t* __restrict__ ids,
                                     const bf16* __restrict__ dy,
                                     float* __restrict__ dtable,
                                     int B, int E) {
    int idx = blockIdx.x * blockDim.x + threadIdx.x;
    if (idx >= B * E) return;
    int b = idx / E, e = idx % E;
    atomicAdd(dtable + ids[b] * E + e, bf2f(dy[idx]));
}

at::Tensor embedding_fwd(at::Tensor ids, at::Tensor table) {
    CHECK_GPU(ids); CHECK_CONTIG(ids);
    CHECK_GPU(table); CHECK_CONTIG(table); CHECK_BF16(table);
    TORCH_CHECK(ids.scalar_type() == at::kLong, "ids must be int64");
    int B = ids.numel(), E = table.size(1);
    auto out = at::empty({B, E}, table.options());
    hipStream_t s = at::cuda::getCurrentCUDAStream();
    hipLaunchKernelGGL(embedding_fwd_kernel, dim3(cdiv(B * E, 256)),
                       dim3(256), 0, s,
                       (const int64_t*)ids.data_ptr(),
                       (const bf16*)table.data_ptr(),
                       (bf16*)out.data_ptr(), B, E);
    HIP_OK(hipGetLastError());
    return out;
}

at::Tensor embedding_bwd(at::Tensor ids, at::Tensor dy, int64_t rows) {
    CHECK_GPU(ids); CHECK_GPU(dy); CHECK_CONTIG(dy); CHECK_BF16(dy);
    int B = ids.numel(), E = dy.size(1);
    auto dtable = at::zeros({rows, E}, dy.options().dtype(at::kFloat));
    hipStream_t s = at::cuda::getCurrentCUDAStream();
    hipLaunchKernelGGL(embedding_bwd_kernel, dim3(cdiv(B * E, 256)),
                       dim3(256), 0, s,
                       (const int64_t*)ids.data_ptr(),
                       (const bf16*)dy.data_ptr(),
                       (float*)dtable.data_ptr(), B, E);
    HIP_OK(hipGetLastError());
    return dtable;
}


__global__ void ce_fwd_kernel(const bf16* __restrict__ logits,
                              const int64_t* __restrict__ labels,
                              const float* __restrict__ mask,
                              float* __restrict__ losses,
                              float* __restrict__ lse,
                              int V) {
    __shared__ float red[8];
    int b = blockIdx.x;
    int tid = threadIdx.x;
    const bf16* row = logits + (int64_t)b * V;

    float lmax = -1e30f;
    for (int v = tid; v < V; v += blockDim.x)
        lmax = fmaxf(lmax, bf2f(row[v]));
    lmax = wave_max(lmax);
    if ((tid & 63) == 0) red[tid >> 6] = lmax;
    __syncthreads();
    float m = -1e30f;
    for (int w = 0; w < (int)(blockDim.x >> 6); ++w) m = fmaxf(m, red[w]);
    __syncthreads();

    float lsum = 0.f;
    for (int v = tid; v < V; v += blockDim.x)
        lsum += __expf(bf2f(row[v]) - m);
    lsum = wave_sum(lsum);
    if ((tid & 63) == 0) red[tid >> 6] = lsum;
    __syncthreads();
    if (tid == 0) {
        float z = 0.f;
        for (int w = 0; w < (int)(blockDim.x >> 6); ++w) z += red[w];
        float l = m + __logf(z);
        lse[b] = l;
        losses[b] = (l - bf2f(row[labels[b]])) * mask[b];
    }
}

__global__ void ce_bwd_kernel(const bf16* __restrict__ logits,
                              const int64_t* __restrict__ labels,
                              const float* __restrict__ mask,
                              const float* __restrict__ lse,
                              const float* __restrict__ dloss,
                              bf16* __restrict__ dlogits,
                              int B, int V) {
    int64_t idx = (int64_t)blockIdx.x * blockDim.x + threadIdx.x;
    if (idx >= (int64_t)B * V) return;
    int b = idx / V, v = idx % V;
    float p = __expf(bf2f(logits[idx]) - lse[b]);
    float g = (p - (labels[b] == v ? 1.f : 0.f)) * mask[b] * dloss[b];
    dlogits[idx] = f2bf(g);
}

std::vector<at::Tensor> ce_fwd(at::Tensor logits, at::Tensor labels,
                               at::Tensor mask) {
    CHECK_GPU(logits); CHECK_CONTIG(logits); CHECK_BF16(logits);
    CHECK_GPU(labels); CHECK_GPU(mask); CHECK_F32(mask);
    int B = logits.size(0), V = logits.size(1);
    auto losses = at::empty({B}, logits.options().dtype(at::kFloat));
    auto lse = at::empty({B}, logits.options().dtype(at::kFloat));
    hipStream_t s = at::cuda::getCurrentCUDAStream();
    hipLaunchKernelGGL(ce_fwd_kernel, dim3(B), dim3(256), 0, s,
                       (const bf16*)logits.data_ptr(),
                       (const int64_t*)labels.data_ptr(),
                       (const float*)mask.data_ptr(),
                       (float*)losses.data_ptr(), (float*)lse.data_ptr(), V);
    HIP_OK(hipGetLastError());
    return {losses, lse};
}

at::Tensor ce_bwd(at::Tensor logits, at::Tensor labels, at::Tensor mask,
                  at::Tensor lse, at::Tensor dloss) {
    CHECK_GPU(logits); CHECK_CONTIG(logits); CHECK_BF16(logits);
    int B = logits.size(0), V = logits.size(1);
    auto dlogits = at::empty_like(logits);
    hipStream_t s = at::cuda::getCurrentCUDAStream();
    hipLaunchKernelGGL(ce_bwd_kernel,
                       dim3(cdiv((int64_t)B * V, 256)), dim3(256), 0, s,
                       (const bf16*)logits.data_ptr(),
                       (const int64_t*)labels.data_ptr(),
                       (const float*)mask.data_ptr(),
                       (const float*)lse.data_ptr(),
                       (const float*)dloss.data_ptr(),
                       (bf16*)dlogits.data_ptr(), B, V);
    HIP_OK(hipGetLastError());
    return dlogits;
}


__global__ void sq_norm_kernel(const float* __restrict__ g, int64_t n,
                               float* __restrict__ out) {
    int64_t idx = (int64_t)blockIdx.x * blockDim.x + threadIdx.x;
    float acc = 0.f;
    for (int64_t i = idx; i < n; i += (int64_t)gridDim.x * blockDim.x)
        acc += g[i] * g[i];
    acc = wave_sum(acc);
    __shared__ float red[8];
    if ((threadIdx.x & 63) == 0) red[threadIdx.x >> 6] = acc;
    __syncthreads();
    if (threadIdx.x == 0) {
        float t = 0.f;
        for (int w = 0; w < (int)(blockDim.x >> 6); ++w) t += red[w];
        atomicAdd(out, t);
    }
}

__global__ void adam_kernel(float* __restrict__ p, const float* __restrict__ g,
                            float* __restrict__ m, float* __restrict__ v,
                            const float* __restrict__ gsq,
                            const float* __restrict__ step_dev,
                            int64_t n, float lr0, float decay_factor,
                            float steps_per_decay, float b1, float b2,
                            float eps, float clip) {
    float step = *step_dev;
    float bc1 = 1.f - powf(b1, step);
    float bc2 = 1.f - powf(b2, step);
    float lr = lr0;
    if (decay_factor < 1.f)
        lr = lr0 * powf(decay_factor, floorf(step / steps_per_decay));
    float scale = 1.f;
    if (clip > 0.f) {
        float norm = sqrtf(*gsq);
        if (norm > clip) scale = clip / norm;
    }
    int64_t idx = (int64_t)blockIdx.x * blockDim.x + threadIdx.x;
    for (int64_t i = idx; i < n; i += (int64_t)gridDim.x * blockDim.x) {
        float gi = g[i] * scale;
        float mi = b1 * m[i] + (1.f - b1) * gi;
        float vi = b2 * v[i] + (1.f - b2) * gi * gi;
        m[i] = mi;
        v[i] = vi;
        float mhat = mi / bc1;
        float vhat = vi / bc2;
        p[i] -= lr * mhat / (sqrtf(vhat) + eps);
    }
}

at::Tensor grad_sq_norm(std::vector<at::Tensor> grads) {
    TORCH_CHECK(!grads.empty());
    auto out = at::zeros({1}, grads[0].options().dtype(at::kFloat));
    hipStream_t s = at::cuda::getCurrentCUDAStream();
    for (auto& g : grads) {
        CHECK_GPU(g); CHECK_CONTIG(g); CHECK_F32(g);
        int64_t n = g.numel();
        int blocks = (int)std::min<int64_t>(cdiv(n, 256), 1024);
        hipLaunchKernelGGL(sq_norm_kernel, dim3(blocks), dim3(256), 0, s,
                           (const float*)g.data_ptr(), n,
                           (float*)out.data_ptr());
    }
    HIP_OK(hipGetLastError());
    return out;
}

void adam_step(std::vector<at::Tensor> params, std::vector<at::Tensor> grads,
               std::vector<at::Tensor> ms, std::vector<at::Tensor> vs,
               at::Tensor step_dev, double lr0, double decay_factor,
               double steps_per_decay, double b1, double b2, double eps,
               double clip, at::Tensor gsq) {
    CHECK_GPU(step_dev); CHECK_F32(step_dev);
    hipStream_t s = at::cuda::getCurrentCUDAStream();
    for (size_t i = 0; i < params.size(); ++i) {
        auto& p = params[i];
        CHECK_GPU(p); CHECK_CONTIG(p); CHECK_F32(p);
        int64_t n = p.numel();
        int blocks = (int)std::min<int64_t>(cdiv(n, 256), 2048);
        hipLaunchKernelGGL(adam_kernel, dim3(blocks), dim3(256), 0, s,
                           (float*)p.data_ptr(),
                           (const float*)grads[i].data_ptr(),
                           (float*)ms[i].data_ptr(), (float*)vs[i].data_ptr(),
                           (const float*)gsq.data_ptr(),
                           (const float*)step_dev.data_ptr(), n,
                           (float)lr0, (float)decay_factor,
                           (float)steps_per_decay, (float)b1, (float)b2,
                           (float)eps, (float)clip);
    }
    HIP_OK(hipGetLastError());
}


__global__ void sq_norm_mt_kernel(const int64_t* __restrict__ desc,
                                  const int64_t* __restrict__ cum,
                                  int n_tensors, int64_t total,
                                  float* __restrict__ out) {
    extern __shared__ int64_t scum[];
    for (int i = threadIdx.x; i <= n_tensors; i += blockDim.x)
        scum[i] = cum[i];
    __syncthreads();
    float acc = 0.f;
    int64_t idx = (int64_t)blockIdx.x * blockDim.x + threadIdx.x;
    int64_t stride = (int64_t)gridDim.x * blockDim.x;
    for (int64_t i = idx; i < total; i += stride) {
        int lo = 0, hi = n_tensors;
        while (hi - lo > 1) {
            int mid = (lo + hi) >> 1;
            if (i >= scum[mid]) lo = mid; else hi = mid;
        }
        const float* g = (const float*)desc[lo * 5 + 1];
        float gv = g[i - scum[lo]];
        acc += gv * gv;
    }
    acc = wave_sum(acc);
    __shared__ float red[4];
    if ((threadIdx.x & 63) == 0) red[threadIdx.x >> 6] = acc;
    __syncthreads();
    if (threadIdx.x == 0)
        atomicAdd(out, red[0] + red[1] + red[2] + red[3]);
}

at::Tensor sq_norm_mt(at::Tensor desc, at::Tensor cum, int64_t n_tensors,
                      int64_t total) {
    auto out = at::zeros({1}, at::TensorOptions()
                                  .dtype(at::kFloat)
                                  .device(desc.device()));
    hipStream_t s = at::cuda::getCurrentCUDAStream();
    int blocks = (int)std::min<int64_t>(cdiv(total, 256 * 8), 2048);
    size_t shm = (n_tensors + 1) * sizeof(int64_t);
    hipLaunchKernelGGL(sq_norm_mt_kernel, dim3(blocks), dim3(256), shm, s,
                       (const int64_t*)desc.data_ptr(),
                       (const int64_t*)cum.data_ptr(),
                       (int)n_tensors, total, (float*)out.data_ptr());
    HIP_OK(hipGetLastError());
    return out;
}

typedef __attribute__((ext_vector_type(4))) float floatx4v;

template <int VEC4>
__global__ void adam_mt_kernel(const int64_t* __restrict__ desc,
                               const int64_t* __restrict__ cum,
                               int n_tensors, int64_t total,
                               const float* __restrict__ gsq,
                               const float* __restrict__ step_dev,
                               float lr0, float decay_factor,
                               float steps_per_decay, float b1, float b2,
                               float eps, float clip, int zero_g) {
    extern __shared__ int64_t scum[];
    for (int i = threadIdx.x; i <= n_tensors; i += blockDim.x)
        scum[i] = cum[i];
    __syncthreads();
    float step = *step_dev;
    float bc1 = 1.f - powf(b1, step);
    float bc2 = 1.f - powf(b2, step);
    float lr = lr0;
    if (decay_factor < 1.f)
        lr = lr0 * powf(decay_factor, floorf(step / steps_per_decay));
    float scale = 1.f;
    if (clip > 0.f) {
        float norm = sqrtf(*gsq);
        if (norm > clip) scale = clip / norm;
    }
    constexpr int V = VEC4 ? 4 : 1;
    int64_t idx = (int64_t)blockIdx.x * blockDim.x + threadIdx.x;
    int64_t stride = (int64_t)gridDim.x * blockDim.x;
    int64_t niter = (total + V - 1) / V;
    for (int64_t it = idx; it < niter; it += stride) {
        int64_t i = it * V;
        int lo = 0, hi = n_tensors;
        while (hi - lo > 1) {
            int mid = (lo + hi) >> 1;
            if (i >= scum[mid]) lo = mid; else hi = mid;
        }
        int64_t off = i - scum[lo];
        float* p = (float*)desc[lo * 5 + 0];
        float* g = (float*)desc[lo * 5 + 1];
        float* m = (float*)desc[lo * 5 + 2];
        float* v = (float*)desc[lo * 5 + 3];
        bf16* sh = (bf16*)desc[lo * 5 + 4];
        if (VEC4) {
            floatx4v g4 = *(floatx4v*)(g + off);
            floatx4v m4 = *(floatx4v*)(m + off);
            floatx4v v4 = *(floatx4v*)(v + off);
            floatx4v p4 = *(floatx4v*)(p + off);
#pragma unroll
            for (int e = 0; e < 4; ++e) {
                float gi = g4[e] * scale;
                float mi = b1 * m4[e] + (1.f - b1) * gi;
                float vi = b2 * v4[e] + (1.f - b2) * gi * gi;
                m4[e] = mi;
                v4[e] = vi;
                p4[e] -= lr * (mi / bc1) / (sqrtf(vi / bc2) + eps);
            }
            *(floatx4v*)(m + off) = m4;
            *(floatx4v*)(v + off) = v4;
            *(floatx4v*)(p + off) = p4;
            if (sh != nullptr) {
#pragma unroll
                for (int e = 0; e < 4; ++e)
                    sh[off + e] = f2bf(p4[e]);
            }
            if (zero_g)
                *(floatx4v*)(g + off) = floatx4v{0.f, 0.f, 0.f, 0.f};
        } else {
            float gi = g[off] * scale;
            float mi = b1 * m[off] + (1.f - b1) * gi;
            float vi = b2 * v[off] + (1.f - b2) * gi * gi;
            m[off] = mi;
            v[off] = vi;
            float pn = p[off]
                - lr * (mi / bc1) / (sqrtf(vi / bc2) + eps);
            p[off] = pn;
            if (sh != nullptr) sh[off] = f2bf(pn);
            if (zero_g) g[off] = 0.f;
        }
    }
}

void adam_step_mt(at::Tensor desc, at::Tensor cum, int64_t n_tensors,
                  int64_t total, at::Tensor step_dev, double lr0,
                  double decay_factor, double steps_per_decay, double b1,
                  double b2, double eps, double clip, at::Tensor gsq,
                  bool zero_grads, bool vec4) {
    hipStream_t s = at::cuda::getCurrentCUDAStream();
    int blocks = (int)std::min<int64_t>(cdiv(total, 256 * 4), 4096);
    size_t shm = (n_tensors + 1) * sizeof(int64_t);
    if (vec4)
        hipLaunchKernelGGL((adam_mt_kernel<1>), dim3(blocks), dim3(256),
                           shm, s,
                           (const int64_t*)desc.data_ptr(),
                           (const int64_t*)cum.data_ptr(),
                           (int)n_tensors, total,
                           (const float*)gsq.data_ptr(),
                           (const float*)step_dev.data_ptr(),
                           (float)lr0, (float)decay_factor,
                           (float)steps_per_decay, (float)b1, (float)b2,
                           (float)eps, (float)clip, zero_grads ? 1 : 0);
    else
        hipLaunchKernelGGL((adam_mt_kernel<0>), dim3(blocks), dim3(256),
                           shm, s,
                           (const int64_t*)desc.data_ptr(),
                           (const int64_t*)cum.data_ptr(),
                           (int)n_tensors, total,
                           (const float*)gsq.data_ptr(),
                           (const float*)step_dev.data_ptr(),
                           (float)lr0, (float)decay_factor,
                           (float)steps_per_decay, (float)b1, (float)b2,
                           (float)eps, (float)clip, zero_grads ? 1 : 0);
    HIP_OK(hipGetLastError());
}
```

Measured before the change: 6024 images/sec.

## Template slab counts, hoist loads, unroll skinny GEMM and attention backward rows

Templates the split-K slab-sum epilogues and the fused LSTM backward/expand kernels on the slab count, so slab loads unroll and are issued up front. It also switches index math to 32-bit and hoists global loads ahead of arithmetic. The skinny MFMA GEMM loop gains multi-step K unrolling with clamped, branch-free addressing, and the attention pool backward processes 8 rows per wave with a compile-time dctx flag. This raises memory-level parallelism and cuts branching in many small latency-bound kernels, at the cost of more registers, more template instantiations and a new 2^31 element limit.

```diff
diff --git a/sat_amd/ops/csrc/bptt_fuse.hip b/sat_amd/ops/csrc/bptt_fuse.hip
--- a/sat_amd/ops/csrc/bptt_fuse.hip
+++ b/sat_amd/ops/csrc/bptt_fuse.hip
@@ -397,6 +397,7 @@
 }
 
 
+template <int S>
 __global__ void dexp_lstm_bwd_kernel(const bf16* __restrict__ dexpd,
                                      const bf16* __restrict__ d_out_carry,
                                      const bf16* __restrict__ d_sth_carry,
@@ -415,41 +416,52 @@
                                      int carry_splitk, int carry_salt) {
     const uint32_t seed = (uint32_t)(*seed_p);
     const int W = H + D + E;
-    int64_t idx = (int64_t)blockIdx.x * blockDim.x + threadIdx.x;
-    if (idx >= (int64_t)B * W) return;
-    int b = idx / W, j = idx % W;
+    int idx = blockIdx.x * blockDim.x + threadIdx.x;
+    if (idx >= B * W) return;
+    int b = idx / W, j = idx - b * W;
     float dexp = bf2f(dexpd[idx])
         * drop_scale(seed, s + 6, (uint32_t)(b * W + j), p_fc);
     if (j < H) {
-        uint32_t hidx = (uint32_t)(b * H + j);
+        const int hi = b * H + j;
+        uint32_t hidx = (uint32_t)hi;
+        float cs[S > 0 ? S : 1];
+        bf16 cb = {};
+        if constexpr (S > 0) load_slabs<S>(carry_slabs, B * H, hi, cs);
+        if constexpr (S < 0) cb = d_out_carry[hi];
+        bf16 sc = d_sth_carry[hi];
+        const bf16* gp = gates + b * 4 * H + j;
+        bf16 gb[4];
+#pragma unroll
+        for (int q = 0; q < 4; ++q) gb[q] = gp[q * H];
+        bf16 cv = c[hi];
+        bf16 dcb = (dc != nullptr ? dc : c)[hi];
+
         float doc;
-        if (carry_slabs != nullptr) {
-            float v = sum_slabs(carry_slabs, (int64_t)B * H,
-                                (int64_t)b * H + j, carry_splitk);
+        if constexpr (S >= 0) {
+            float v;
+            if constexpr (S > 0) v = add_slabs<S>(cs);
+            else v = sum_slabs<0>(carry_slabs, B * H, hi, carry_splitk);
             v *= drop_scale(seed, carry_salt, hidx, p_fc);
             doc = bf2f(f2bf(v));
         } else {
-            doc = bf2f(d_out_carry[(int64_t)b * H + j]);
+            doc = bf2f(cb);
         }
         float dout = dexp + doc;
         float dhv = dout * drop_scale(seed, s + 4, hidx, p_lstm)
-            + bf2f(d_sth_carry[(int64_t)b * H + j])
-            * drop_scale(seed, s + 5, hidx, p_lstm);
-        const bf16* gp = gates + (int64_t)b * 4 * H + j;
+            + bf2f(sc) * drop_scale(seed, s + 5, hidx, p_lstm);
         float g[4], dg[4], dcp;
 #pragma unroll
-        for (int q = 0; q < 4; ++q) g[q] = bf2f(gp[q * H]);
-        float dcv = (dc != nullptr) ? bf2f(dc[(int64_t)b * H + j]) : 0.f;
-        lstm_cell_bwd(g, bf2f(c[(int64_t)b * H + j]), dhv, dcv, fb, dg,
-                      dcp);
-        bf16* dgp = dgates + (int64_t)b * 4 * H + j;
+        for (int q = 0; q < 4; ++q) g[q] = bf2f(gb[q]);
+        float dcv = (dc != nullptr) ? bf2f(dcb) : 0.f;
+        lstm_cell_bwd(g, bf2f(cv), dhv, dcv, fb, dg, dcp);
+        bf16* dgp = dgates + b * 4 * H + j;
 #pragma unroll
         for (int q = 0; q < 4; ++q) dgp[q * H] = f2bf(dg[q]);
-        dc_prev[(int64_t)b * H + j] = f2bf(dcp);
+        dc_prev[hi] = f2bf(dcp);
     } else if (j < H + D) {
-        dpool_dec[(int64_t)b * D + (j - H)] = f2bf(dexp);
+        dpool_dec[b * D + (j - H)] = f2bf(dexp);
     } else {
-        demb_dec[(int64_t)b * E + (j - H - D)] = f2bf(dexp);
+        demb_dec[b * E + (j - H - D)] = f2bf(dexp);
     }
 }
 
@@ -470,21 +482,30 @@
     if (dc.defined() && dc.numel() > 0)
         dc_ptr = (const bf16*)dc.data_ptr();
     int64_t n = (int64_t)B * (H + D + E);
+    TORCH_CHECK(n < (1LL << 31) && (int64_t)B * 4 * H < (1LL << 31),
+                "expand row or gates have >= 2^31 elements");
     hipStream_t st = at::cuda::getCurrentCUDAStream();
-    hipLaunchKernelGGL(dexp_lstm_bwd_kernel, dim3(cdiv(n, 256)),
-                       dim3(256), 0, st,
-                       (const bf16*)dexpd.data_ptr(), carry_ptr,
-                       (const bf16*)d_sth_carry.data_ptr(),
-                       (const int64_t*)seed.data_ptr(),
-                       (const bf16*)gates.data_ptr(),
-                       (const bf16*)c_prev.data_ptr(), dc_ptr,
-                       (bf16*)dgates_out.data_ptr(),
-                       (bf16*)dc_prev.data_ptr(),
-                       (bf16*)dpool_dec.data_ptr(),
-                       (bf16*)demb_dec.data_ptr(),
-                       B, H, (int)D, (int)E,
-                       (float)p_fc, (float)p_lstm, (int)s, (float)fb,
-                       slab_ptr, carry_splitk, (int)carry_salt);
+#define LAUNCH_DEXP(S) \
+    hipLaunchKernelGGL(dexp_lstm_bwd_kernel<S>, dim3(cdiv(n, 256)), \
+                       dim3(256), 0, st, \
+                       (const bf16*)dexpd.data_ptr(), carry_ptr, \
+                       (const bf16*)d_sth_carry.data_ptr(), \
+                       (const int64_t*)seed.data_ptr(), \
+                       (const bf16*)gates.data_ptr(), \
+                       (const bf16*)c_prev.data_ptr(), dc_ptr, \
+                       (bf16*)dgates_out.data_ptr(), \
+                       (bf16*)dc_prev.data_ptr(), \
+                       (bf16*)dpool_dec.data_ptr(), \
+                       (bf16*)demb_dec.data_ptr(), \
+                       B, H, (int)D, (int)E, \
+                       (float)p_fc, (float)p_lstm, (int)s, (float)fb, \
+                       slab_ptr, carry_splitk, (int)carry_salt)
+    if (slab_ptr == nullptr) {
+        LAUNCH_DEXP(-1);
+    } else {
+        SLAB_DISPATCH(carry_splitk, LAUNCH_DEXP)
+    }
+#undef LAUNCH_DEXP
     HIP_OK(hipGetLastError());
     return {dc_prev, dpool_dec, demb_dec};
 }
diff --git a/sat_amd/ops/csrc/common.h b/sat_amd/ops/csrc/common.h
--- a/sat_amd/ops/csrc/common.h
+++ b/sat_amd/ops/csrc/common.h
@@ -193,10 +193,44 @@
                          .memory_format(at::MemoryFormat::ChannelsLast));
 }
 
+constexpr int MAX_SLABS = 8;
+
+template <int S>
+__device__ __forceinline__ void load_slabs(const float* __restrict__ Yf,
+                                           int64_t n, int64_t off,
+                                           float (&s)[S > 0 ? S : 1]) {
+#pragma unroll
+    for (int k = 0; k < S; ++k) s[k] = Yf[k * n + off];
+}
+
+template <int S>
+__device__ __forceinline__ float add_slabs(const float (&s)[S > 0 ? S : 1]) {
+    float v = 0.f;
+#pragma unroll
+    for (int k = 0; k < S; ++k) v += s[k];
+    return v;
+}
+
+template <int S>
 __device__ __forceinline__ float sum_slabs(const float* __restrict__ Yf,
                                            int64_t n, int64_t off,
                                            int splitk) {
-    float v = 0.f;
-    for (int k = 0; k < splitk; ++k) v += Yf[k * n + off];
-    return v;
-}
+    if constexpr (S > 0) {
+        float s[S];
+        load_slabs<S>(Yf, n, off, s);
+        return add_slabs<S>(s);
+    } else {
+        float v = 0.f;
+        for (int k = 0; k < splitk; ++k) v += Yf[k * n + off];
+        return v;
+    }
+}
+
+#define SLAB_DISPATCH(splitk, CALL) \
+    switch (splitk) { \
+        case 1: CALL(1); break; case 2: CALL(2); break; \
+        case 3: CALL(3); break; case 4: CALL(4); break; \
+        case 5: CALL(5); break; case 6: CALL(6); break; \
+        case 7: CALL(7); break; case 8: CALL(8); break; \
+        default: CALL(0); break; \
+    }
diff --git a/sat_amd/ops/csrc/gemm.hip b/sat_amd/ops/csrc/gemm.hip
--- a/sat_amd/ops/csrc/gemm.hip
+++ b/sat_amd/ops/csrc/gemm.hip
@@ -170,53 +170,66 @@
     for (int i = 0; i < RF; ++i)
         acc[i] = floatx4{0.f, 0.f, 0.f, 0.f};
 
-    const bool wfull = (n0 + 16 <= N);
     if (active) {
-        for (int k = kbeg; k < kend; k += 32) {
-            const int kof = k + kgrp * 8;
-            bf16x8 b_frag = {};
-            if (kof + 8 <= K) {
-                int gb = n0 + lrow;
-                if (wfull || gb < N)
-                    b_frag = *(const bf16x8*)(W + (int64_t)gb * K + kof);
-            } else if (kof < K) {
-                int gb = n0 + lrow;
-                if (wfull || gb < N)
-                    for (int e = 0; e < 8 && kof + e < K; ++e)
-                        b_frag[e] = W[(int64_t)gb * K + kof + e];
+        const bf16* wp = W + (int64_t)min(n0 + lrow, N - 1) * K + kgrp * 8;
+        int64_t aoff[RF];
+#pragma unroll
+        for (int mi = 0; mi < RF; ++mi)
+            aoff[mi] = (int64_t)min(mi * 16 + lrow, M - 1) * K + kgrp * 8;
+        const bool pre = TANHA && blockIdx.x == 0 && wave == 0;
+
+        auto steps = [&](auto uc, int k) {
+            constexpr int U = decltype(uc)::value;
+            bf16x8 bw[U], a[U][RF];
+            floatx4 g0[TANHA ? U : 1][RF], g1[TANHA ? U : 1][RF];
+#pragma unroll
+            for (int u = 0; u < U; ++u) {
+                bw[u] = *(const bf16x8*)(wp + k + u * 32);
+#pragma unroll
+                for (int mi = 0; mi < RF; ++mi) {
+                    const int64_t ao = aoff[mi] + k + u * 32;
+                    if constexpr (TANHA) {
+                        g0[u][mi] = *(const floatx4*)(Af + ao);
+                        g1[u][mi] = *(const floatx4*)(Af + ao + 4);
+                        a[u][mi] = *(const bf16x8*)(Ay + ao);
+                    } else {
+                        a[u][mi] = *(const bf16x8*)(A + ao);
+                    }
+                }
             }
 #pragma unroll
-            for (int mi = 0; mi < RF; ++mi) {
-                bf16x8 a0 = {};
-                int ar = mi * 16 + lrow;
-                if constexpr (TANHA) {
-                    if (ar < M) {
-                        const int64_t ao = (int64_t)ar * K + kof;
-                        floatx4 g0 = *(const floatx4*)(Af + ao);
-                        floatx4 g1 = *(const floatx4*)(Af + ao + 4);
-                        bf16x8 yv = *(const bf16x8*)(Ay + ao);
+            for (int u = 0; u < U; ++u)
+#pragma unroll
+                for (int mi = 0; mi < RF; ++mi) {
+                    if constexpr (TANHA) {
+                        bf16x8 yv = a[u][mi];
 #pragma unroll
                         for (int e = 0; e < 8; ++e) {
                             float y = bf2f(yv[e]);
-                            float g = e < 4 ? g0[e] : g1[e - 4];
-                            a0[e] = f2bf(g * (1.f - y * y));
+                            float g = e < 4 ? g0[u][mi][e]
+                                            : g1[u][mi][e - 4];
+                            a[u][mi][e] = f2bf(g * (1.f - y * y));
                         }
-                        if (blockIdx.x == 0 && wave == 0)
-                            *(bf16x8*)(Apre + ao) = a0;
+                        if (pre && mi * 16 + lrow < M)
+                            *(bf16x8*)(Apre + aoff[mi] + k + u * 32)
+                                = a[u][mi];
                     }
-                } else
-                if (kof + 8 <= K) {
-                    if (ar < M)
-                        a0 = *(const bf16x8*)(A + (int64_t)ar * K + kof);
-                } else if (kof < K) {
-                    if (ar < M)
-                        for (int e = 0; e < 8 && kof + e < K; ++e)
-                            a0[e] = A[(int64_t)ar * K + kof + e];
+                    acc[mi] = __builtin_amdgcn_mfma_f32_16x16x32_bf16(
+                        a[u][mi], bw[u], acc[mi], 0, 0, 0);
                 }
-                acc[mi] = __builtin_amdgcn_mfma_f32_16x16x32_bf16(
-                    a0, b_frag, acc[mi], 0, 0, 0);
-            }
-        }
+        };
+
+        constexpr int U = TANHA ? (RF >= 8 ? 1 : 8 / RF)
+                                : (RF >= 8 ? 2 : 12 / RF);
+        int k = kbeg;
+        for (; k + U * 32 <= kend; k += U * 32)
+            steps(std::integral_constant<int, U>{}, k);
+        if constexpr (U > 2)
+            for (; k + 64 <= kend; k += 64)
+                steps(std::integral_constant<int, 2>{}, k);
+        if constexpr (U > 1)
+            for (; k < kend; k += 32)
+                steps(std::integral_constant<int, 1>{}, k);
     }
 
     const int col = n0 + (lane & 15);
@@ -246,6 +259,7 @@
         }
 }
 
+template <int S>
 __global__ void skinny_epilogue_kernel(const float* __restrict__ Yf,
                                        const bf16* __restrict__ bias,
                                        bf16* __restrict__ Y,
@@ -253,8 +267,10 @@
                                        int splitk) {
     int64_t idx = (int64_t)blockIdx.x * blockDim.x + threadIdx.x;
     if (idx >= n) return;
-    float v = sum_slabs(Yf, n, idx, splitk);
-    if (bias != nullptr) v += bf2f(bias[idx % N]);
+    const bf16* bp = bias != nullptr ? bias + idx % N : (const bf16*)Yf;
+    float bv = bf2f(*bp);
+    float v = sum_slabs<S>(Yf, n, idx, splitk);
+    if (bias != nullptr) v += bv;
     Y[idx] = f2bf(apply_act(v, act));
 }
 
@@ -353,10 +369,14 @@
 static void launch_epilogue(hipStream_t stream, const at::Tensor& yf,
                             const bf16* bias, at::Tensor& y, int act) {
     int64_t n = y.numel();
-    hipLaunchKernelGGL(skinny_epilogue_kernel, dim3(cdiv(n, 256)),
-                       dim3(256), 0, stream, (const float*)yf.data_ptr(),
-                       bias, (bf16*)y.data_ptr(), n, (int)y.size(1), act,
-                       (int)yf.size(0));
+    const int splitk = (int)yf.size(0);
+#define LAUNCH_EPI(S) \
+    hipLaunchKernelGGL(skinny_epilogue_kernel<S>, dim3(cdiv(n, 256)), \
+                       dim3(256), 0, stream, (const float*)yf.data_ptr(), \
+                       bias, (bf16*)y.data_ptr(), n, (int)y.size(1), act, \
+                       splitk)
+    SLAB_DISPATCH(splitk, LAUNCH_EPI)
+#undef LAUNCH_EPI
 }
 
 at::Tensor dense_fwd(at::Tensor x, at::Tensor w, at::Tensor bias,
@@ -423,15 +443,31 @@
 }
 
 
+template <int S>
 __global__ void skinny_epilogue_drop_kernel(
         const float* __restrict__ Yf, bf16* __restrict__ Y,
         const int64_t* __restrict__ seed_p, int64_t n, int splitk,
         float p, int salt) {
     int64_t idx = (int64_t)blockIdx.x * blockDim.x + threadIdx.x;
     if (idx >= n) return;
-    float v = sum_slabs(Yf, n, idx, splitk);
+    float v = sum_slabs<S>(Yf, n, idx, splitk);
     v *= drop_scale((uint32_t)(*seed_p), salt, (uint32_t)idx, p);
     Y[idx] = f2bf(v);
+}
+
+static void launch_epilogue_drop(hipStream_t stream, const at::Tensor& yf,
+                                 at::Tensor& y, const at::Tensor& seed,
+                                 double p, int64_t salt) {
+    int64_t n = y.numel();
+    const int splitk = (int)yf.size(0);
+#define LAUNCH_EPI(S) \
+    hipLaunchKernelGGL(skinny_epilogue_drop_kernel<S>, \
+                       dim3(cdiv(n, 256)), dim3(256), 0, stream, \
+                       (const float*)yf.data_ptr(), (bf16*)y.data_ptr(), \
+                       (const int64_t*)seed.data_ptr(), n, splitk, \
+                       (float)p, (int)salt)
+    SLAB_DISPATCH(splitk, LAUNCH_EPI)
+#undef LAUNCH_EPI
 }
 
 at::Tensor dense_fwd_drop(at::Tensor x, at::Tensor w, at::Tensor seed,
@@ -446,12 +482,7 @@
     auto y = at::empty({M, N}, x.options());
     hipStream_t stream = at::cuda::getCurrentCUDAStream();
     auto yf = skinny_slabs(stream, x, w);
-    int64_t n = M * N;
-    hipLaunchKernelGGL(skinny_epilogue_drop_kernel,
-                       dim3(cdiv(n, 256)), dim3(256), 0, stream,
-                       (const float*)yf.data_ptr(), (bf16*)y.data_ptr(),
-                       (const int64_t*)seed.data_ptr(), n,
-                       (int)yf.size(0), (float)p, (int)salt);
+    launch_epilogue_drop(stream, yf, y, seed, p, salt);
     HIP_OK(hipGetLastError());
     return y;
 }
@@ -462,34 +493,46 @@
     TORCH_CHECK(yf.dim() == 3, "slabs must be [splitk, M, N]");
     auto y = at::empty({yf.size(1), yf.size(2)},
                        yf.options().dtype(at::kBFloat16));
-    int64_t n = y.numel();
     hipStream_t stream = at::cuda::getCurrentCUDAStream();
-    hipLaunchKernelGGL(skinny_epilogue_drop_kernel,
-                       dim3(cdiv(n, 256)), dim3(256), 0, stream,
-                       (const float*)yf.data_ptr(), (bf16*)y.data_ptr(),
-                       (const int64_t*)seed.data_ptr(), n,
-                       (int)yf.size(0), (float)p, (int)salt);
+    launch_epilogue_drop(stream, yf, y, seed, p, salt);
     HIP_OK(hipGetLastError());
     return y;
 }
 
 
+template <int S>
 __device__ __forceinline__ void sum_gates(const float* __restrict__ Yf,
                                           const bf16* __restrict__ bias,
+                                          const bf16* __restrict__ c_prev,
                                           bf16* __restrict__ gates,
                                           int B, int H, int b, int hh,
-                                          int splitk, float g[4]) {
-    int64_t n = (int64_t)B * 4 * H;
+                                          int splitk, float g[4],
+                                          float& cp) {
+    const int n = B * 4 * H;
+    const int off0 = b * 4 * H + hh;
+    const bf16* bp = bias != nullptr ? bias + hh : c_prev;
+    const int bstride = bias != nullptr ? H : 0;
+    float s[4][S > 0 ? S : 1];
+    bf16 bv[4];
+    if constexpr (S > 0) {
+#pragma unroll
+        for (int q = 0; q < 4; ++q) load_slabs<S>(Yf, n, off0 + q * H, s[q]);
+    }
+#pragma unroll
+    for (int q = 0; q < 4; ++q) bv[q] = bp[q * bstride];
+    cp = bf2f(c_prev[b * H + hh]);
 #pragma unroll
     for (int q = 0; q < 4; ++q) {
-        int64_t off = (int64_t)b * 4 * H + q * H + hh;
-        float acc = sum_slabs(Yf, n, off, splitk);
-        if (bias != nullptr) acc += bf2f(bias[q * H + hh]);
-        gates[off] = f2bf(acc);
+        float acc;
+        if constexpr (S > 0) acc = add_slabs<S>(s[q]);
+        else acc = sum_slabs<0>(Yf, n, off0 + q * H, splitk);
+        if (bias != nullptr) acc += bf2f(bv[q]);
+        gates[off0 + q * H] = f2bf(acc);
         g[q] = acc;
     }
 }
 
+template <int S>
 __global__ void skinny_epi_lstm_kernel(const float* __restrict__ Yf,
                                        const bf16* __restrict__ bias,
                                        const bf16* __restrict__ c_prev,
@@ -500,9 +543,10 @@
                                        float fb) {
     int idx = blockIdx.x * blockDim.x + threadIdx.x;
     if (idx >= B * H) return;
-    float g[4], cn, h;
-    sum_gates(Yf, bias, gates, B, H, idx / H, idx % H, splitk, g);
-    lstm_cell_fwd(g, bf2f(c_prev[idx]), fb, cn, h);
+    float g[4], cp, cn, h;
+    sum_gates<S>(Yf, bias, c_prev, gates, B, H, idx / H, idx % H, splitk,
+                 g, cp);
+    lstm_cell_fwd(g, cp, fb, cn, h);
     h_out[idx] = f2bf(h);
     c_out[idx] = f2bf(cn);
 }
@@ -517,15 +561,19 @@
     auto h_out = at::empty_like(c_prev);
     auto c_out = at::empty_like(c_prev);
     hipStream_t s = at::cuda::getCurrentCUDAStream();
+    TORCH_CHECK(M * N < (1LL << 31), "gates have >= 2^31 elements");
     auto yf = skinny_slabs(s, xh, wl);
-    hipLaunchKernelGGL(skinny_epi_lstm_kernel,
-                       dim3(cdiv(B * H, 256)), dim3(256), 0, s,
-                       (const float*)yf.data_ptr(),
-                       (const bf16*)bl.data_ptr(),
-                       (const bf16*)c_prev.data_ptr(),
-                       (bf16*)gates.data_ptr(), (bf16*)h_out.data_ptr(),
-                       (bf16*)c_out.data_ptr(), B, H, (int)yf.size(0),
-                       (float)fb);
+    const int splitk = (int)yf.size(0);
+#define LAUNCH_EPI(S) \
+    hipLaunchKernelGGL(skinny_epi_lstm_kernel<S>, \
+                       dim3(cdiv(B * H, 256)), dim3(256), 0, s, \
+                       (const float*)yf.data_ptr(), \
+                       (const bf16*)bl.data_ptr(), \
+                       (const bf16*)c_prev.data_ptr(), \
+                       (bf16*)gates.data_ptr(), (bf16*)h_out.data_ptr(), \
+                       (bf16*)c_out.data_ptr(), B, H, splitk, (float)fb)
+    SLAB_DISPATCH(splitk, LAUNCH_EPI)
+#undef LAUNCH_EPI
     HIP_OK(hipGetLastError());
     return {gates, h_out, c_out};
 }
@@ -638,6 +686,7 @@
 }
 
 
+template <int S>
 __global__ void skinny_epi_dx_kernel(const float* __restrict__ Yf,
                                      const bf16* __restrict__ dpool_dec,
                                      const bf16* __restrict__ demb_dec,
@@ -645,26 +694,29 @@
                                      bf16* __restrict__ dpooled,
                                      bf16* __restrict__ demb_out,
                                      bf16* __restrict__ dsth,
-                                     int64_t n, int splitk,
+                                     int n, int splitk,
                                      int B, int D, int E, int H,
                                      float p, int salt) {
     const uint32_t seed = (uint32_t)(*seed_p);
     const int I = D + E;
     const int W = I + H;
-    int64_t idx = (int64_t)blockIdx.x * blockDim.x + threadIdx.x;
+    int idx = blockIdx.x * blockDim.x + threadIdx.x;
     if (idx >= n) return;
-    float g = sum_slabs(Yf, n, idx, splitk);
-    int b = (int)(idx / W), j = (int)(idx % W);
+    int b = idx / W, j = idx - b * W;
+    const bf16* addp = j < D ? dpool_dec + b * D + j
+                     : j < I ? demb_dec + b * E + (j - D)
+                             : (const bf16*)Yf;
+    float add = bf2f(*addp);
+    float g = sum_slabs<S>(Yf, n, idx, splitk);
     if (j < I) {
+#pragma clang fp contract(off)
         g *= drop_scale(seed, salt, (uint32_t)(b * I + j), p);
         if (j < D)
-            dpooled[(int64_t)b * D + j] =
-                f2bf(g + bf2f(dpool_dec[(int64_t)b * D + j]));
+            dpooled[b * D + j] = f2bf(g + add);
         else
-            demb_out[(int64_t)b * E + (j - D)] =
-                f2bf(g + bf2f(demb_dec[(int64_t)b * E + (j - D)]));
+            demb_out[b * E + (j - D)] = f2bf(g + add);
     } else {
-        dsth[(int64_t)b * H + (j - I)] = f2bf(g);
+        dsth[b * H + (j - I)] = f2bf(g);
     }
 }
 
@@ -684,22 +736,28 @@
     hipStream_t stream = at::cuda::getCurrentCUDAStream();
     auto yf = skinny_slabs(stream, dgates, wl_t);
     int64_t n = M * N;
-    hipLaunchKernelGGL(skinny_epi_dx_kernel, dim3(cdiv(n, 256)),
-                       dim3(256), 0, stream,
-                       (const float*)yf.data_ptr(),
-                       (const bf16*)dpool_dec.data_ptr(),
-                       (const bf16*)demb_dec.data_ptr(),
-                       (const int64_t*)seed.data_ptr(),
-                       (bf16*)dpooled.data_ptr(),
-                       (bf16*)demb_out.data_ptr(),
-                       (bf16*)dsth.data_ptr(),
-                       n, (int)yf.size(0), (int)M, (int)D, (int)E, (int)H,
-                       (float)p, (int)salt);
+    TORCH_CHECK(n < (1LL << 31), "dxh has >= 2^31 elements");
+    const int splitk = (int)yf.size(0);
+#define LAUNCH_EPI(S) \
+    hipLaunchKernelGGL(skinny_epi_dx_kernel<S>, dim3(cdiv(n, 256)), \
+                       dim3(256), 0, stream, \
+                       (const float*)yf.data_ptr(), \
+                       (const bf16*)dpool_dec.data_ptr(), \
+                       (const bf16*)demb_dec.data_ptr(), \
+                       (const int64_t*)seed.data_ptr(), \
+                       (bf16*)dpooled.data_ptr(), \
+                       (bf16*)demb_out.data_ptr(), \
+                       (bf16*)dsth.data_ptr(), \
+                       (int)n, splitk, (int)M, (int)D, (int)E, (int)H, \
+                       (float)p, (int)salt)
+    SLAB_DISPATCH(splitk, LAUNCH_EPI)
+#undef LAUNCH_EPI
     HIP_OK(hipGetLastError());
     return {dpooled, dsth};
 }
 
 
+template <int S, bool XN>
 __global__ void skinny_epi_lstm_expand_kernel(
         const float* __restrict__ Yf, const bf16* __restrict__ bias,
         const bf16* __restrict__ c_prev,
@@ -717,35 +775,40 @@
     const uint32_t seed = (uint32_t)(*seed_p);
     const int W = H + D + E;
     const int I = D + E;
-    int64_t idx = (int64_t)blockIdx.x * blockDim.x + threadIdx.x;
-    if (idx >= (int64_t)B * W) return;
-    int b = idx / W, j = idx % W;
+    int idx = blockIdx.x * blockDim.x + threadIdx.x;
+    if (idx >= B * W) return;
+    int b = idx / W, j = idx - b * W;
     float val;
     if (j < H) {
-        float g[4], cn, h;
-        sum_gates(Yf, bias, gates, B, H, b, j, splitk, g);
-        lstm_cell_fwd(g, bf2f(c_prev[(int64_t)b * H + j]), fb, cn, h);
-        c_out[(int64_t)b * H + j] = f2bf(cn);
+        float g[4], cp, cn, h;
+        sum_gates<S>(Yf, bias, c_prev, gates, B, H, b, j, splitk, g, cp);
+        lstm_cell_fwd(g, cp, fb, cn, h);
+        c_out[b * H + j] = f2bf(cn);
         uint32_t hidx = (uint32_t)(b * H + j);
         float ot = h * drop_scale(seed, s + 4, hidx, p_lstm);
         bf16 sth = f2bf(h * drop_scale(seed, s + 5, hidx, p_lstm));
-        sth_t[(int64_t)b * H + j] = sth;
-        if (xh_next != nullptr)
-            xh_next[(int64_t)b * W + I + j] = sth;
+        sth_t[b * H + j] = sth;
+        if constexpr (XN)
+            xh_next[b * W + I + j] = sth;
         if (od_next != nullptr)
-            od_next[(int64_t)b * H + j] =
+            od_next[b * H + j] =
                 f2bf(ot * drop_scale(seed, s + 16 + 1, hidx, p_fc));
         val = ot;
     } else if (j < H + D) {
-        val = bf2f(pooled[(int64_t)b * D + (j - H)]);
+        val = bf2f(pooled[b * D + (j - H)]);
     } else {
         int e = j - H - D;
-        val = bf2f(table[ids[b] * E + e]);
-        if (xh_next != nullptr)
-            xh_next[(int64_t)b * W + D + e] =
-                f2bf(bf2f(table[next_ids[b] * E + e])
+        int64_t id = ids[b], nid = 0;
+        if constexpr (XN) nid = next_ids[b];
+        bf16 tv = table[id * E + e];
+        if constexpr (XN) {
+            bf16 tn = table[nid * E + e];
+            xh_next[b * W + D + e] =
+                f2bf(bf2f(tn)
                      * drop_scale(seed, s + 16 + 3,
                                   (uint32_t)(b * I + D + e), p_lstm));
+        }
+        val = bf2f(tv);
     }
     expdrop[idx] = f2bf(val * drop_scale(seed, s + 6,
                                          (uint32_t)(b * W + j), p_fc));
@@ -773,21 +836,29 @@
     if (od_next.defined() && od_next.numel() > 0)
         od_ptr = (bf16*)od_next.data_ptr();
     int64_t n = (int64_t)B * (H + D + E);
-    hipLaunchKernelGGL(skinny_epi_lstm_expand_kernel,
-                       dim3(cdiv(n, 256)), dim3(256), 0, stream,
-                       (const float*)yf.data_ptr(), bias_ptr,
-                       (const bf16*)c_prev.data_ptr(),
-                       (const bf16*)pooled.data_ptr(),
-                       (const bf16*)table.data_ptr(),
-                       (const int64_t*)ids.data_ptr(),
-                       (const int64_t*)seed.data_ptr(),
-                       (bf16*)gates.data_ptr(),
-                       (bf16*)c_out.data_ptr(),
-                       (bf16*)sth_t.data_ptr(),
-                       (bf16*)expdrop.data_ptr(), od_ptr,
-                       B, H, D, E, (int)yf.size(0),
-                       (float)fb, (float)p_lstm, (float)p_fc, (int)s,
-                       next_ids_ptr, xh_next_ptr);
+    TORCH_CHECK(n < (1LL << 31) && M * N < (1LL << 31),
+                "expand row or gates have >= 2^31 elements");
+    const int splitk = (int)yf.size(0);
+#define LAUNCH_EPI(S) \
+    hipLaunchKernelGGL((xh_next_ptr != nullptr \
+                            ? skinny_epi_lstm_expand_kernel<S, true> \
+                            : skinny_epi_lstm_expand_kernel<S, false>), \
+                       dim3(cdiv(n, 256)), dim3(256), 0, stream, \
+                       (const float*)yf.data_ptr(), bias_ptr, \
+                       (const bf16*)c_prev.data_ptr(), \
+                       (const bf16*)pooled.data_ptr(), \
+                       (const bf16*)table.data_ptr(), \
+                       (const int64_t*)ids.data_ptr(), \
+                       (const int64_t*)seed.data_ptr(), \
+                       (bf16*)gates.data_ptr(), \
+                       (bf16*)c_out.data_ptr(), \
+                       (bf16*)sth_t.data_ptr(), \
+                       (bf16*)expdrop.data_ptr(), od_ptr, \
+                       B, H, D, E, splitk, \
+                       (float)fb, (float)p_lstm, (float)p_fc, (int)s, \
+                       next_ids_ptr, xh_next_ptr)
+    SLAB_DISPATCH(splitk, LAUNCH_EPI)
+#undef LAUNCH_EPI
     HIP_OK(hipGetLastError());
     return {gates, c_out, sth_t};
 }
diff --git a/sat_amd/ops/csrc/kernels.hip b/sat_amd/ops/csrc/kernels.hip
--- a/sat_amd/ops/csrc/kernels.hip
+++ b/sat_amd/ops/csrc/kernels.hip
@@ -224,11 +224,15 @@
 }
 
 
-__global__ void attn_pool_bwd_p1_kernel(
+
+template <bool DCTX>
+__global__ __launch_bounds__(256)
+void attn_pool_bwd_p1_kernel(
         const bf16* __restrict__ ctx, const float* __restrict__ alpha,
         const bf16* __restrict__ dpooled,
         float* __restrict__ sbuf, bf16* __restrict__ dctx,
         int L, int D) {
+    constexpr int R = 8;
     int b = blockIdx.x;
     int nchunk = gridDim.y;
     int lchunk = (L + nchunk - 1) / nchunk;
@@ -238,30 +242,43 @@
     const bf16* cb = ctx + (int64_t)b * L * D;
     const bf16* dp = dpooled + (int64_t)b * D;
 
-    for (int l = l0 + wid; l < l1; l += 4) {
-        float acc = 0.f;
-        float a = alpha[(int64_t)b * L + l];
+    for (int lb = l0 + wid; lb < l1; lb += 4 * R) {
+        float a[R], acc[R];
+        const bf16* cr[R];
+#pragma unroll
+        for (int r = 0; r < R; ++r) {
+            int l = min(lb + 4 * r, l1 - 1);
+            a[r] = alpha[(int64_t)b * L + l];
+            cr[r] = cb + (int64_t)l * D;
+            acc[r] = 0.f;
+        }
         for (int d0 = lane * 8; d0 + 8 <= D; d0 += 64 * 8) {
-            bf16x8 cv = *(const bf16x8*)(cb + (int64_t)l * D + d0);
+            bf16x8 cv[R];
+#pragma unroll
+            for (int r = 0; r < R; ++r)
+                cv[r] = *(const bf16x8*)(cr[r] + d0);
             bf16x8 dv = *(const bf16x8*)(dp + d0);
-            if (dctx != nullptr) {
+#pragma unroll
+            for (int r = 0; r < R; ++r) {
                 bf16x8 out;
 #pragma unroll
                 for (int e = 0; e < 8; ++e) {
                     float dpe = bf2f(dv[e]);
-                    acc += bf2f(cv[e]) * dpe;
-                    out[e] = f2bf(a * dpe);
+                    acc[r] += bf2f(cv[r][e]) * dpe;
+                    if constexpr (DCTX) out[e] = f2bf(a[r] * dpe);
                 }
-                *(bf16x8*)(dctx + (int64_t)b * L * D + (int64_t)l * D + d0)
-                    = out;
-            } else {
-#pragma unroll
-                for (int e = 0; e < 8; ++e)
-                    acc += bf2f(cv[e]) * bf2f(dv[e]);
+                if constexpr (DCTX) {
+                    if (lb + 4 * r < l1)
+                        *(bf16x8*)(dctx + (cr[r] - ctx) + d0) = out;
+                }
             }
         }
-        acc = wave_sum(acc);
-        if (lane == 0) sbuf[(int64_t)b * L + l] = acc;
+#pragma unroll
+        for (int r = 0; r < R; ++r) {
+            float s = wave_sum(acc[r]);
+            if (lane == 0 && lb + 4 * r < l1)
+                sbuf[(int64_t)b * L + lb + 4 * r] = s;
+        }
     }
 }
 
@@ -272,11 +289,14 @@
     __shared__ float red[4];
     int b = blockIdx.x;
     int tid = threadIdx.x;
+    const float* dap = dalpha != nullptr ? dalpha : sbuf;
     float part = 0.f;
     for (int l = tid; l < L; l += blockDim.x) {
         float da = sbuf[(int64_t)b * L + l];
-        if (dalpha != nullptr) da += dalpha[(int64_t)b * L + l];
-        part += alpha[(int64_t)b * L + l] * da;
+        float dx = dap[(int64_t)b * L + l];
+        float al = alpha[(int64_t)b * L + l];
+        if (dalpha != nullptr) da += dx;
+        part += al * da;
     }
     part = wave_sum(part);
     if ((tid & 63) == 0) red[tid >> 6] = part;
@@ -284,9 +304,10 @@
     float dot = red[0] + red[1] + red[2] + red[3];
     for (int l = tid; l < L; l += blockDim.x) {
         float da = sbuf[(int64_t)b * L + l];
-        if (dalpha != nullptr) da += dalpha[(int64_t)b * L + l];
-        dlogits[(int64_t)b * L + l] =
-            alpha[(int64_t)b * L + l] * (da - dot);
+        float dx = dap[(int64_t)b * L + l];
+        float al = alpha[(int64_t)b * L + l];
+        if (dalpha != nullptr) da += dx;
+        dlogits[(int64_t)b * L + l] = al * (da - dot);
     }
 }
 
@@ -311,7 +332,9 @@
     if (dalpha.defined() && dalpha.numel() > 0)
         dalpha_ptr = (const float*)dalpha.data_ptr();
     hipStream_t s = at::cuda::getCurrentCUDAStream();
-    hipLaunchKernelGGL(attn_pool_bwd_p1_kernel, dim3(B, 8), dim3(256), 0, s,
+    hipLaunchKernelGGL((need_dctx ? attn_pool_bwd_p1_kernel<true>
+                                  : attn_pool_bwd_p1_kernel<false>),
+                       dim3(B, 8), dim3(256), 0, s,
                        (const bf16*)ctx.data_ptr(),
                        (const float*)alpha.data_ptr(),
                        (const bf16*)dpooled.data_ptr(),
```

Result: faster. 6602 images/sec (median of 6 runs) (+9.6%).
